# DTUWindEnergy/WindGym

Hardware: AMD Instinct MI355X
Metric: env-steps/sec (whole node), 16-turbine farm x 4096 envs (higher is better)
Workload: dtype f32

## Files before the change

### windgym_amd/csrc/wg_env.hip

```cpp
#include <hip/hip_runtime.h>

#ifndef WG_ENV_ABLATE
#define WG_ENV_ABLATE 0
#endif
#include "wg_env_common.h"
#include "wg_internal.h"

struct __attribute__((aligned(16))) EnvSlotLds {
    int dev_rem, fill_rem, sub, budget;
    double s_new;
    int n_emit, n_valid, new_valid;
    unsigned n_emitted;
    float s_off_f, near_f, move_max, ti_pow;
    double s_off, ws;
    float ws_f, ti_f, wd_env, base_acc;
    int n_pushed, pend_farm_n, pend_base_n, n_flow;
    double c_time;
    int c_head;
    unsigned c_part, c_flow, c_istep, c_tag, n_emitted0;
    float out_pw;
    unsigned c_add;
    int bg_init;
    int pad_[3];
};
static_assert(sizeof(EnvSlotLds) == WG_ENV_SLOT_LDS_BYTES, "keep WG_ENV_SLOT_LDS_BYTES in sync (wg_flow.h)");
#define WG_ENV_OFF_SRC4 0
#define WG_ENV_OFF_REC4 1024
#define WG_ENV_OFF_RING 2048
#define WG_ENV_OFF_XR 3072
#define WG_ENV_OFF_SRC2 3584
#define WG_ENV_OFF_SL 4096
#define WG_ENV_OFF_HDR (WG_ENV_OFF_SL + 4 * WG_ENV_SLOT_LDS_BYTES)
#define WG_ENV_OFF_STAGE (WG_ENV_OFF_HDR + 128)
static_assert(WG_ENV_OFF_STAGE == WG_ENV_FIXED_LDS_BYTES, "keep WG_ENV_FIXED_LDS_BYTES in sync (wg_flow.h)");

__device__ __forceinline__ float env_slot_sums(const float v, const int N, const int NS, const int k, const int tid) {
    if (N == 16) return wg_row_sum(v);
    if (N < 16) {
        const int r = tid >> 4, i = tid & 15;
        const float x = __shfl(v, (r * N + i) & 63, 64);
        const float s = wg_row_sum((i < N && r < NS) ? x : 0.f);
        return __shfl(s, k << 4, 64);
    }
    const int h = tid >> 5, i = tid & 31;
    const float x = __shfl(v, (h * N + i) & 63, 64);
    float s = (i < N && h < NS) ? x : 0.f;
    WG_ROW_REDUCE(s, wg_addf)
    s += __shfl_xor(s, 16, 64);
    return __shfl(s, k << 5, 64);
}

static __device__ __forceinline__ void env_clone_dev(char* const smem, const int kd, const int N, const int P, const double dt_d,
                                                               float* const py_env, unsigned* const ra_env, const unsigned src,
                                                               const unsigned dst, const int lane) {
    float4* const Lsrc4 = reinterpret_cast<float4*>(smem + WG_ENV_OFF_SRC4);
    int4* const Lring = reinterpret_cast<int4*>(smem + WG_ENV_OFF_RING);
    float2* const Lsrc2 = reinterpret_cast<float2*>(smem + WG_ENV_OFF_SRC2);
    EnvSlotLds* const SL = reinterpret_cast<EnvSlotLds*>(smem + WG_ENV_OFF_SL);
    const int ga = (kd - 1) * N, gb = kd * N;
    const int4 last = Lring[ga + N - 1];
    const int nq = (last.x + last.y) >> 2;
    {
        const float4* const ps = reinterpret_cast<const float4*>(py_env + src);
        float4* const pd = reinterpret_cast<float4*>(py_env + dst);
        const uint4* const rs = reinterpret_cast<const uint4*>(ra_env + 2 * (size_t)src);
        uint4* const rd = reinterpret_cast<uint4*>(ra_env + 2 * (size_t)dst);
#pragma unroll 2
        for (int q = lane; q < nq; q += 64) {
            const float4 y = ps[q];
            const uint4 r0 = rs[q], r1 = rs[q + nq];
            pd[q] = y; rd[q] = r0; rd[q + nq] = r1;
        }
    }
    if (lane < N) {
        Lsrc4[gb + lane] = Lsrc4[ga + lane];
        Lsrc2[gb + lane] = Lsrc2[ga + lane];
        Lring[gb + lane].z = Lring[ga + lane].z;
    }
    if (lane == 0) {
        const EnvSlotLds& a = SL[kd - 1];
        EnvSlotLds& b = SL[kd];
        b.n_valid = a.n_valid; b.n_emitted = a.n_emitted; b.s_off = a.s_off;
        b.dev_rem = 0; b.sub = 0;
        b.budget = a.budget;
        double tm = a.c_time;
        for (int i = 0; i < a.n_flow; ++i) tm += dt_d;
        b.c_time = tm;
        int hd = a.c_head + (int)((a.n_emitted - a.n_emitted0) % (unsigned)P); if (hd >= P) hd -= P;
        b.c_head = hd; b.n_emitted0 = a.n_emitted;
        b.c_istep = a.c_istep + (unsigned)a.n_flow;
    }
}

template <bool NOISE, int WPE, int GLUE, int SPLIT>
__device__ __forceinline__ void env_flow(char* const smem, char* const smem_pass, float* const zone, const int wv, const int role, const int mode,
                                         const float* __restrict__ actions, const uint8_t* __restrict__ mask, const int chunk, EnvFlowOut& out) {
    const int tid = threadIdx.x & 63, e = blockIdx.x;
    int N, F, NS, NL;
    float inv_N;
    {
        const KArgsPtr ka = wg_cold_args();
        N = ka->p.N; F = ka->p.F; inv_N = ka->p.inv_N;
        NS = WPE == 2 ? F : 2 * F; NL = NS * N;
    }
    const int kbase = WPE == 2 ? wv * F : 0;
    const bool valid = tid < NL;
    const int g = valid ? tid : 0;
    const int k = (int)(((float)g + 0.5f) * inv_N);
    const int t = g - k * N;
    const int c = WPE == 2 ? wv : (F == 2 ? (k >> 1) : k), farm = F == 2 ? (k & 1) : 0;

    float4* const Lsrc4 = reinterpret_cast<float4*>(smem + WG_ENV_OFF_SRC4);
    uint4* const Lrec4 = reinterpret_cast<uint4*>(smem + WG_ENV_OFF_REC4);
    int4* const Lring = reinterpret_cast<int4*>(smem + WG_ENV_OFF_RING);
    double* const Lxr = reinterpret_cast<double*>(smem + WG_ENV_OFF_XR);
    float2* const Lsrc2 = reinterpret_cast<float2*>(smem + WG_ENV_OFF_SRC2);
    EnvSlotLds* const SL = reinterpret_cast<EnvSlotLds*>(smem + WG_ENV_OFF_SL);
    float* const def = reinterpret_cast<float*>(smem + WG_ENV_OFF_STAGE);
    float* const tiav = def + WG_ENV_CAP;
    unsigned short* const cl = reinterpret_cast<unsigned short*>(tiav + WG_ENV_CAP);
    unsigned short* const ql = reinterpret_cast<unsigned short*>(smem + WG_ENV_OFF_STAGE);
    EnvSlotLds& my = SL[k];

    WG_STAMP(0);
    typedef const __attribute__((address_space(4))) WgEnv* CEnvPtr;
    int env_live;
    bool role_live = false, role_dev = false, defer_init = false, split_on = false;
    bool parked = false;
    float yaw, tu, tti, oyaw;
    {
        const KArgsPtr k0 = wg_cold_args();
        static_assert(sizeof(WgEnv) == 128, "the env header is loaded as 32 words");
        const int hw = reinterpret_cast<const int*>(k0->d.env + e)[tid & 31];
        if (GLUE != 0 && tid < 32) reinterpret_cast<int*>(smem + WG_ENV_OFF_HDR)[tid] = hw;
        out.bg_init_pending = 0; out.rounds = 0; out.first_obs = 0;
        const bool use_mask = mode == WG_MODE_RESET && mask != nullptr;
        const uint8_t mask_byte = *(use_mask ? mask + e : reinterpret_cast<const uint8_t*>(k0->d.env + e));
        const bool masked_out = use_mask && mask_byte == 0;
        const unsigned ctx_id = (unsigned)(e * 2 + c), slot_id = (unsigned)(e * 2 * F + kbase + k);
        const unsigned tb = (unsigned)((e * 2 * F + kbase) * N + g);
        const unsigned tcx = ctx_id * (unsigned)N + (unsigned)t;

        int dev_rem, fill_rem, n_pushed, pend_farm_n, pend_base_n, init_pending, time_max_c, n_valid, c_head;
        unsigned n_emitted, c_part, c_flow, c_istep, c_tag, c_add;
        double s_off, ws, l_xr, l_yr, c_time;
        float ti_f, wd_env, l_yaw, l_u, l_ti, l_act;
        float4 l_bnd;
        int l_roff, l_rnext;
        auto load_state = [&]() __attribute__((always_inline)) {
            const KArgsPtr kl = wg_cold_args();
            const WgSlot& slot = kl->d.slot[slot_id];
            const WgCtx& cx = kl->d.ctx[ctx_id];
            dev_rem = slot.dev_remaining; fill_rem = slot.fill_remaining;
            s_off = slot.s_off; c_time = slot.time; c_head = slot.head; n_valid = slot.n_valid; c_istep = slot.istep;
            n_emitted = slot.n_emitted; c_part = slot.part_count; c_flow = slot.flow_count; c_add = slot.add_count;
            ws = cx.ws; ti_f = (float)cx.ti; wd_env = (float)cx.wd;
            n_pushed = cx.n_pushed; pend_farm_n = cx.pend_farm_n; pend_base_n = cx.pend_base_n;
            c_tag = (unsigned)cx.episode_tag; init_pending = cx.init_pending; time_max_c = cx.time_max;
            const int* ro = kl->d.roff + ctx_id * (unsigned)(N + 1);
            l_roff = ro[(unsigned)t]; l_rnext = ro[(unsigned)t + 1u];
            l_xr = kl->d.xr[tcx]; l_yr = kl->d.yr[tcx];
            l_yaw = kl->d.yaw[tb]; l_u = kl->d.u[tb]; l_ti = kl->d.ti_loc[tb];
            l_bnd = reinterpret_cast<const float4*>(kl->d.bnd)[tb];
        };
        load_state();
        const int n_tab = k0->p.n_tab, S = k0->p.S;
        const unsigned i_tab = (unsigned)min(tid, n_tab - 1), i_s = (unsigned)min(tid, S - 1);
        const float pf_tp = k0->d.tab_power[i_tab], pf_tc = k0->d.tab_ct[i_tab];
        const float pf_dy = k0->d.rotor_dy[i_s], pf_dz = k0->d.rotor_dz[i_s];
        {
            const bool has_act = mode == WG_MODE_STEP && farm == 0;
            const float a = *(has_act ? actions + (unsigned)(e * N + t) : k0->d.tab_ct);
            l_act = has_act ? a : 0.f;
        }

#define WG_HDR_I(f) __builtin_amdgcn_readlane(hw, (int)(offsetof(WgEnv, f) / 4))
        env_live = WG_HDR_I(live);
        int env_done = WG_HDR_I(done), env_shadow_iters = WG_HDR_I(shadow_iters), env_steps_done = WG_HDR_I(steps_done);
        int env_timestep = WG_HDR_I(timestep), env_time_max_live = WG_HDR_I(time_max_live);
#undef WG_HDR_I
        if (SPLIT && role == 1) {
            if (tid == 0) { *reinterpret_cast<int*>(smem + WG_ENV_OFF_HDR) = 0; if (GLUE != 0 && (SPLIT == 1 || wv == 0)) reinterpret_cast<int*>(zone)[LEAN_PRE_FLAG] = 0; }
            asm volatile("s_waitcnt vmcnt(0) lgkmcnt(0)" ::: "memory");
        }
        if (WPE == 2) {
            asm volatile("" : "+s"(env_live), "+s"(env_done), "+s"(env_shadow_iters), "+s"(env_steps_done), "+s"(env_timestep), "+s"(env_time_max_live) : : "memory");
            asm volatile("s_barrier" ::: "memory");
        }
        if (SPLIT && role == 1 && GLUE != 0 && c == env_live) {
            const EnvKArgsPtr kz = (EnvKArgsPtr)wg_cold_args();
            const LeanEarly zr = lean_early_load(*(const WgParams*)&kz->gp, *(const WgPtrs*)&kz->gd, e, N, F, tid, hw);
            double* const zs = reinterpret_cast<double*>(zone);
#pragma unroll
            for (int sI = 0; sI < WG_N_CH; ++sI) { zs[LEAN_PRE_S(sI, tid)] = zr.S[sI]; zone[LEAN_PRE_LV(sI, tid)] = zr.lv[sI]; }
            zone[LEAN_PRE_MET(tid)] = zr.met;
            if (tid == 0) { zone[LEAN_PRE_FOLD] = zr.f_old; zone[LEAN_PRE_BOLD] = zr.b_old; }
            asm volatile("s_waitcnt lgkmcnt(0)" ::: "memory");
            if (tid == 0) env_flag_set(reinterpret_cast<int*>(zone) + LEAN_PRE_FLAG);
        }
        out.env_live = env_live;
        out.truncates = env_timestep >= env_time_max_live;
        out.steps_done = env_steps_done; out.time_max_live = env_time_max_live;

        const bool is_live_c = (c == env_live);
        const int autoreset = k0->p.autoreset;
        int budget = 0;
        long plan_left = 0;
        if (mode == WG_MODE_STEP) {
            role_live = is_live_c && !env_done;
            role_dev = !is_live_c && autoreset != 0;
            const int bg_pending = WPE == 2 ? (is_live_c ? 0 : __shfl(init_pending, 0, 64)) : __shfl(init_pending, (env_live ^ 1) * F * N, 64);
            out.bg_init_pending = autoreset && bg_pending;
            if (SPLIT == 2 && role == 1 && out.bg_init_pending) return;
            if (autoreset && bg_pending && WPE == 1 && !out.truncates) {
                defer_init = true;
                budget = 0;
            } else if (autoreset && bg_pending) {
                const KArgsPtr ki = wg_cold_args();
                const WgParams& gp = *ki->d.gp;
                env_init_episode<GLUE != 0>(e, env_live ^ 1, tid);
                full_barrier<64>();
                load_state();
                const int fill_max = F == 2 ? max(gp.fill_a, gp.fill_b) : gp.fill_a;
                const int tm = WPE == 2 ? ki->d.ctx[e * 2 + env_live].time_max : __shfl(time_max_c, env_live * F * N, 64);
                const long total = wg_rule_episode_steps(tm, gp.extra_inc);
                const int dev0 = __shfl(dev_rem, WPE == 2 ? 0 : (env_live ^ 1) * F * N, 64);
                budget = wg_shadow_share(dev0 + gp.K * fill_max, total - env_steps_done, env_steps_done, e);
                budget = wg_shadow_share(dev_rem + gp.K * fill_rem, total - env_steps_done, env_steps_done, e, farm ? 0x80000000u : 0u);
                plan_left = total - env_steps_done;
            } else {
                const long total = wg_rule_episode_steps_inc(env_time_max_live, k0->p.env_inc);
                budget = role_dev ? wg_shadow_share(dev_rem + k0->p.K * fill_rem, total - env_steps_done, env_steps_done, e, farm ? 0x80000000u : 0u) : 0;
                plan_left = total - env_steps_done;
            }
        } else {
            role_dev = is_live_c && !masked_out;
            budget = chunk;
        }
        bool clone_here = false;
        if (k0->p.env_share) {
            const int dev_a = __shfl(dev_rem, (tid - N) & 63, 64);
            parked = valid && role_dev && farm == 1 && dev_rem > 0 && c_istep == 0u && dev_a > 0;
            const int twin_fill = __shfl(parked ? fill_rem + 1 : 0, (tid + N) & 63, 64);
            const bool lead = valid && role_dev && farm == 0 && twin_fill > 0;
            if (lead && mode == WG_MODE_STEP && !defer_init)
                budget = wg_shadow_share(dev_rem + k0->p.K * max(fill_rem, twin_fill - 1), plan_left, env_steps_done, e);
            if (parked) budget = 0;
            clone_here = lead && budget >= dev_rem;
        }
        if (SPLIT) {
            const bool two = valid && role_dev && budget >= 2;
            split_on = mode == WG_MODE_STEP && k0->p.K == 1 && (is_live_c || (SPLIT == 2 && !out.bg_init_pending)) && !defer_init && !__ballot(two) &&
                       !__ballot(clone_here);
            if (role == 1 && !split_on) return;
        }
        if (WPE == 2 && valid && t == 0) {
            my.dev_rem = dev_rem; my.fill_rem = fill_rem; my.bg_init = out.bg_init_pending; my.n_flow = 0; my.out_pw = 0.f;
        }
        {
            const bool any_work = valid && (role_live || (role_dev && budget > 0 && (dev_rem > 0 || fill_rem > 0)));
            if (!__ballot(any_work)) {
                if (WPE == 2 && mode == WG_MODE_STEP && !is_live_c && autoreset && role == 0) {
                    const int d0 = __shfl(dev_rem, 0, 64), f0 = __shfl(fill_rem, 0, 64), np0 = __shfl(n_pushed, 0, 64);
                    const KArgsPtr kf = wg_cold_args();
                    if (d0 == 0 && f0 == 0 && kf->d.gd->next_obs_ok != nullptr && kf->d.gd->next_obs_ok[ctx_id] == 0) {
                        out.first_obs = 1;
                        env_first_obs<GLUE != 0>((int)ctx_id, np0, tid);
                    }
                }
                return;
            }
        }

        const KArgsPtr k1 = wg_cold_args();
        const int rlen = l_rnext - l_roff;
        const int head = n_emitted == 0u ? rlen - 1 : fast_mod((int)(n_emitted - 1u), rlen, __builtin_amdgcn_rcpf((float)rlen));
        const float ws_f = (float)ws;
        if (valid) {
            Lxr[g] = l_xr;
            Lsrc4[g] = make_float4((float)l_xr, (float)l_yr, l_bnd.y, l_bnd.z);
            Lsrc2[g] = make_float2(l_bnd.x, l_bnd.w);
            Lring[g] = make_int4(l_roff, rlen, head, k);
            Lrec4[g] = make_uint4(0u, 0u, 0u, __float_as_uint(1.f));
            if (t == 0) {
                my.dev_rem = dev_rem; my.fill_rem = fill_rem; my.sub = 0; my.budget = budget;
                my.n_valid = n_valid; my.n_emitted = n_emitted; my.n_emitted0 = n_emitted;
                my.move_max = fabsf(k1->p.hill) * ws_f * k1->p.dt; my.ti_pow = fast_pow(ti_f, k1->p.tic);
                my.s_off = s_off; my.ws = ws; my.ws_f = ws_f; my.ti_f = ti_f; my.wd_env = wd_env; my.base_acc = 0.f;
                my.n_pushed = n_pushed; my.pend_farm_n = pend_farm_n; my.pend_base_n = pend_base_n; my.n_flow = 0;
                my.bg_init = out.bg_init_pending;
                my.c_time = c_time; my.c_head = c_head; my.c_part = c_part; my.c_flow = c_flow; my.c_istep = c_istep; my.c_tag = c_tag; my.c_add = c_add;
            }
        }
        float* const tabp = reinterpret_cast<float*>(smem + k1->p.env_off_tab);
        float* const tabct = tabp + n_tab;
        float2* const rpt = reinterpret_cast<float2*>(tabct + n_tab);
        const float hub = k1->p.hub;
        auto rp = [&](const float dy_, const float dz_) __attribute__((always_inline)) {
            const float dz = hub + dz_ - hub;
            return make_float2(dy_, dz * dz);
        };
        if (tid < n_tab) { tabp[tid] = pf_tp; tabct[tid] = pf_tc; }
        if (tid < S) rpt[tid] = rp(pf_dy, pf_dz);
        for (int i = tid + 64; i < n_tab; i += 64) { tabp[i] = k1->d.tab_power[i]; tabct[i] = k1->d.tab_ct[i]; }
        for (int i = tid + 64; i < S; i += 64) rpt[i] = rp(k1->d.rotor_dy[i], k1->d.rotor_dz[i]);

        yaw = l_yaw; tu = l_u; tti = l_ti; oyaw = l_yaw;
        if (role_live && farm == 0 && valid) {
            yaw = wg_rule_adjust_yaw(k1->p.action_method, yaw, l_act, k1->p.yaw_min, k1->p.yaw_max, k1->p.yaw_step);
        }
    }
    float tpow = 0.f, tct = 0.f, cg = 1.f;
    float sws = 0.f, swd = 0.f, syaw = 0.f, sp_ = 0.f;
    int part_acc = 0, stream_acc = 0;
    bool stepped = false;
    lds_barrier<64>();
    WG_STAMP(1);

    auto glue_early = [&]() __attribute__((always_inline)) {
        if (GLUE != 0 && SPLIT == 0) {
            if (WPE == 2 && wv != env_live) {
                out.g_early = LeanEarly{};
            } else {
                const EnvKArgsPtr kz = (EnvKArgsPtr)wg_cold_args();
                const int hwl = reinterpret_cast<const int*>(smem + WG_ENV_OFF_HDR)[tid & 31];
                out.g_early = lean_early_load(*(const WgParams*)&kz->gp, *(const WgPtrs*)&kz->gd, e, N, F, tid, hwl);
            }
        }
    };
    for (int round = 0;; ++round) {
        bool stepping, is_dev;
        int sub, K;
        if (__ballot(parked)) {
            bool due = parked && SL[k - 1].dev_rem == 0;
            unsigned long long due_m = __ballot(due);
            if (due_m) {
                full_barrier<64>();
                const KArgsPtr kc = wg_cold_args();
                const unsigned pstride = (unsigned)kc->p.pstride;
                const size_t pb_env = (size_t)(e * 2 * F + kbase) * pstride;
                const int src_lane = (tid - N) & 63;
                const float c_tu = __shfl(tu, src_lane, 64), c_tti = __shfl(tti, src_lane, 64), c_pw = __shfl(tpow, src_lane, 64);
                const float c_ct = __shfl(tct, src_lane, 64), c_cg = __shfl(cg, src_lane, 64);
                if (due) { tu = c_tu; tti = c_tti; tpow = c_pw; tct = c_ct; cg = c_cg; stepped = true; parked = false; }
                while (due_m) {
                    const int kd = __builtin_amdgcn_readlane(k, __builtin_ctzll(due_m));
                    env_clone_dev(smem, kd, N, kc->p.P, kc->p.dt_d, kc->d.py + pb_env, kc->d.rec_a + 2 * pb_env, (unsigned)(kd - 1) * pstride,
                                  (unsigned)kd * pstride, tid);
                    due_m &= ~(((1ull << N) - 1ull) << (kd * N));
                }
                lds_barrier<64>();
                glue_early();
            }
        }
        {
            const KArgsPtr kr = wg_cold_args();
            K = kr->p.K;
            const int4 sch = *reinterpret_cast<const int4*>(&my.dev_rem);
            const bool active = sch.x > 0 || sch.y > 0;
            stepping = valid && (role_live ? (round < K) : (role_dev && active && (sch.w > 0 || sch.z != 0)));
            is_dev = !role_live && sch.x > 0;
            sub = sch.z;
            if (!__ballot(stepping)) break;
        out.rounds = round + 1;
            if (round > 0) full_barrier<64>();

            if (role_live && farm == 1 && stepping) {
                const float ystep = kr->p.yaw_step;
                if (kr->p.base_controller == WG_CTRL_LOCAL) {
                    yaw = wg_rule_ctrl_local(yaw, 0.f, ystep);
                } else {
                    yaw = wg_rule_ctrl_global(yaw, ystep);
                }
            }

            if (stepping && t == 0) {
                const double dpart = kr->p.dpart;
                const int P = kr->p.P;
                const double s_off = my.s_off, adv = my.ws * kr->p.dt_d;
                double s_new = s_off + adv;
                int n_emit = 0;
                while (s_new >= dpart) { s_new -= dpart; ++n_emit; }
                if (n_emit > P) n_emit = P;
                int new_valid = my.n_valid + n_emit; if (new_valid > P) new_valid = P;
                my.s_new = s_new; my.n_emit = n_emit; my.new_valid = new_valid;
                my.s_off_f = (float)s_off;
                my.near_f = (float)(s_off + adv + dpart) + 0.01f;
            }
        }
        lds_barrier<64>();
        WG_STAMP(4);

        unsigned cmask = 0u;
        {
            const KArgsPtr kp = wg_cold_args();
            const float D = kp->p.D, inv_D = kp->p.inv_D, eps_max = kp->p.env_eps_max;
            const int gs0 = k * N;
            const float lim0 = kp->p.R_rot + 1.0e-3f * D;
            const float near_f = my.near_f, move_max = my.move_max;
            const float xt_f = Lsrc4[g].x, yt_f = Lsrc4[g].y;
#pragma unroll 4
            for (int s2 = 0; s2 < N; ++s2) {
                const float4 a = Lsrc4[gs0 + s2];
                const float2 b = Lsrc2[gs0 + s2];
                const float dxf = xt_f - a.x;
                const bool nearp = dxf < near_f;
                const float kb_ = nearp ? fmaxf(WG_K_MAX, a.z) : a.z, eb_ = nearp ? fmaxf(eps_max, a.w) : a.w;
                const float sig_max = (kb_ * (dxf * inv_D) + eb_) * D;
                const float bdv = b.x + (((__float_as_uint(b.y) != 0u) | nearp) ? move_max : 0.f);
                const float gap = fabsf(yt_f - a.y) - (5.0f * sig_max + bdv);
                const bool cd = (s2 != t) & (dxf >= 0.f) & (gap <= lim0);
                cmask |= cd ? (1u << s2) : 0u;
            }
            if (!stepping || (SPLIT && role == 1)) cmask = 0u;
        }
        int cbeg, nc;
        {
            const int cnt = __popc(cmask);
            const int inc = wg_wave_scan_i(cnt);
            cbeg = inc - cnt;
            nc = __builtin_amdgcn_readlane(inc, 63);
            unsigned m = cmask;
            int o = cbeg;
            while (m) { cl[o++] = (unsigned short)((g << 5) | __builtin_ctz(m)); m &= m - 1u; }
        }
        lds_barrier<64>();
        WG_STAMP(5);

        struct Cand { uint2 q0, q1; float y0, y1, xd, wgt; int en, jp0; bool ok, rest; };
        float dsum = 0.f, tia_max = 0.f;
        {
            const KArgsPtr kp = wg_cold_args();
            const unsigned pstride = (unsigned)kp->p.pstride;
            const size_t pb_env = (size_t)(e * 2 * F + kbase) * pstride;
            const uint2* const rc_env = reinterpret_cast<const uint2*>(kp->d.rec_a + 2 * pb_env);
            const float* const py_env = kp->d.py + pb_env;
            const double inv_dpart = kp->p.inv_dpart;
            const float inv_D = kp->p.inv_D;
            auto issue = [&](Cand& cd, const int cidx, const int c0, const int c1) __attribute__((always_inline)) {
                cd.ok = false; cd.rest = false;
                if (cidx >= c1) return;
                def[cidx - c0] = 0.f; tiav[cidx - c0] = 0.f;
                const unsigned en = cl[cidx];
                cd.en = (int)en;
                const int gt = (int)(en >> 5);
                const int4 rt = Lring[gt];
                const int gs = rt.w * N + (int)(en & 31u);
                const EnvSlotLds& q = SL[rt.w];
                const double dx = Lxr[gt] - Lxr[gs];
                if (!(dx > 0.0)) return;
                cd.xd = (float)dx * inv_D;
                const double xi = (dx - q.s_new) * inv_dpart;
                const double jf = floor(xi);
                cd.wgt = (float)(xi - jf);
                int j = (int)jf;
                if (j < 0) { j = 0; cd.wgt = 0.f; }
                if (j + 1 > q.new_valid - 1) return;
                const int4 rg = Lring[gs];
                const int Rs = rg.y, hd = rg.z;
                const unsigned mv = __float_as_uint(Lsrc2[gs].y);
                cd.rest = !(mv != 0u && (int)(q.n_emitted - mv) < Rs);
                cd.jp0 = j - q.n_emit;
                int r0 = hd - cd.jp0; if (r0 < 0) r0 += Rs;
                int r1 = hd - cd.jp0 - 1; if (r1 < 0) r1 += Rs;
                if (cd.jp0 < 0) r0 = 0;
                if (cd.jp0 + 1 < 0) r1 = 0;
                const unsigned sb = (unsigned)rg.w * pstride + (unsigned)rg.x;
                cd.q0 = rc_env[sb + (unsigned)r0]; cd.q1 = rc_env[sb + (unsigned)r1];
                cd.y0 = 0.f; cd.y1 = 0.f;
                if (!cd.rest) { cd.y0 = py_env[sb + (unsigned)r0]; cd.y1 = py_env[sb + (unsigned)r1]; }
#if WG_ENV_ABLATE & 1
                cd.q0 = make_uint2(Lrec4[gs].x, Lrec4[gs].y); cd.q1 = cd.q0; cd.y0 = cd.y1 = Lsrc4[gs].y;
#endif
                cd.ok = true;
            };
            Cand ca, cb_;
            issue(ca, tid, 0, min(nc, WG_ENV_CAP));
            WG_STAMP(11);

            if (stepping) {
                const KArgsPtr kq = wg_cold_args();
                const int n_tab = kq->p.n_tab;
                const float* const tabct = reinterpret_cast<const float*>(smem + kq->p.env_off_tab) + n_tab;
                const float gy = yaw * WG_DEG2RAD_F;
                const float sg = __sinf(gy);
                cg = __cosf(gy);
                const float wsn = fmaxf(tu * cg, 0.0f);
                const float ctx = fminf(fmaxf(env_tab(tabct, kq->p.tab_x0, kq->p.tab_inv_dx, n_tab, wsn) * cg * cg, 0.0f), 0.96f);
                const float rq = __builtin_amdgcn_sqrtf(1.0f - ctx);
                const float beta = 0.5f * (1.0f + rq) * __builtin_amdgcn_rcpf(rq);
                const float rk = kq->p.ka * tti + kq->p.kb;
                const float reps = kq->p.eps0 * __builtin_amdgcn_sqrtf(beta);
                const float rhv = -kq->p.hill * sg * tu;
                if (rk > WG_K_MAX || fabsf(rhv) > WG_HV_MAX) atomicOr(kq->d.status, WG_STATUS_BIT_RANGE);
                const unsigned na_ = pack_a(ctx, rk), nb_ = pack_b(tu * __builtin_amdgcn_rcpf(kq->p.ue_scale * my.ws_f), rhv);
                float4 s4 = Lsrc4[g];
                s4.z = fmaxf(s4.z, rk + WG_K_MAX / 65535.0f);
                s4.w = fmaxf(s4.w, reps + 1.0f / 65535.0f);
                Lsrc4[g] = s4;
                const int n_emit = my.n_emit;
                if (n_emit > 0 && rec_moves(nb_)) Lsrc2[g].y = __uint_as_float(my.n_emitted + (unsigned)n_emit);
                Lrec4[g] = make_uint4(na_, nb_, __float_as_uint(tu), __float_as_uint(cg));
            }
            lds_barrier<64>();
            WG_STAMP(2);

            const KArgsPtr ke2 = wg_cold_args();
            const float dpart_f = ke2->p.dpart_f, D = ke2->p.D, dt = ke2->p.dt, R_rot = ke2->p.R_rot, eps0 = ke2->p.eps0, ue_scale = ke2->p.ue_scale;
            const float tia = ke2->p.no_ti_fold ? 0.f : ke2->p.tia, tib = ke2->p.tib, tid_ = ke2->p.tid, inv_S = ke2->p.inv_S;
            const int S = ke2->p.S;
            const float2* const rpt = reinterpret_cast<const float2*>(smem + ke2->p.env_off_tab + 8 * ke2->p.n_tab);
            auto eval_cand = [&](const Cand& cd, const int pos) __attribute__((always_inline)) {
                    if (!cd.ok) return;
#ifdef WG_TIMELINE
                    atomicAdd(&wg_counts[1], 1);
#endif
                    const int gt = cd.en >> 5;
                    const int kt = Lring[gt].w;
                    const int gs = kt * N + (cd.en & 31);
                    const float4 st = Lsrc4[gt];
                    const float ysrc = Lsrc4[gs].y;
                    const EnvSlotLds& q = SL[kt];
                    const int jp0 = cd.jp0, jp1 = jp0 + 1;
                    float py0 = cd.rest ? ysrc : cd.y0, py1 = cd.rest ? ysrc : cd.y1;
                    unsigned a0 = cd.q0.x, b0_ = cd.q0.y, a1 = cd.q1.x, b1_ = cd.q1.y;
                    if (jp0 < 0) {
                        const uint4 rn = Lrec4[gs];
                        py0 = ysrc; a0 = rn.x; b0_ = rn.y;
                        if (jp1 < 0) { py1 = ysrc; a1 = rn.x; b1_ = rn.y; }
                    }
                    const float ue_max = ue_scale * q.ws_f;
                    const float u0 = rec_uf(b0_) * ue_max, u1 = rec_uf(b1_) * ue_max;
                    {
                        const int nv = q.n_valid;
                        const float sof = q.s_off_f;
                        if (!cd.rest && jp0 >= 0 && jp0 < nv) py0 = m0_advect(py0, a0, b0_, jp0, sof, dpart_f, inv_D, dt, eps0);
                        if (!cd.rest && jp1 >= 0 && jp1 < nv) py1 = m0_advect(py1, a1, b1_, jp1, sof, dpart_f, inv_D, dt, eps0);
                    }
                    const float wgt = cd.wgt;
                    const float w0 = 1.0f - wgt, w1 = wgt;
                    const float yc = w0 * py0 + w1 * py1;
                    const float kv = w0 * rec_k(a0) + w1 * rec_k(a1);
                    const float epv = w0 * rec_eps(a0, eps0) + w1 * rec_eps(a1, eps0);
                    const float xd = cd.xd;
                    const float sp = kv * xd + epv;
                    const float sig = sp * D;
                    const float yt = st.y;
                    const float rc2 = (yt - yc) * (yt - yc);
                    const float rcut = R_rot + 5.0f * sig;
                    if (rc2 > rcut * rcut) return;
#ifdef WG_TIMELINE
                    atomicAdd(&wg_counts[2], 1);
                    if (rc2 <= (R_rot + 3.0f * sig) * (R_rot + 3.0f * sig)) atomicAdd(&wg_counts[3], 1);
#endif
                    const float ctv = w0 * rec_ct(a0) + w1 * rec_ct(a1);
                    const float uev = w0 * u0 + w1 * u1;
                    const float inv2s2 = __builtin_amdgcn_rcpf(2.0f * sig * sig);
                    const float cf = m0_cfrac(ctv, sp);
                    const float ind = 0.5f * (1.0f - __builtin_amdgcn_sqrtf(1.0f - ctv));
                    tiav[pos] = tia * fast_pow(ind, tib) * q.ti_pow * fast_pow(fmaxf(xd, 1.0f), tid_) * __expf(-rc2 * inv2s2);
                    const float cgt = __uint_as_float(Lrec4[gt].w), amp = uev * cf;
                    const float ninv = -inv2s2;
                    float acc = 0.f;
#pragma unroll 4
                    for (int sI = 0; sI < ((WG_ENV_ABLATE & 8) ? 1 : S); ++sI) {
                        const float2 rp = rpt[sI];
                        const float dy = yt + rp.x * cgt - yc;
                        acc += amp * __expf((dy * dy + rp.y) * ninv);
                    }
                    def[pos] = acc * inv_S;
            };
#ifdef WG_TIMELINE
            if (tid == 0) atomicAdd(&wg_counts[0], nc);
#endif
            for (int c0 = 0; c0 < nc; c0 += WG_ENV_CAP) {
                const int c1 = min(nc, c0 + WG_ENV_CAP);
                if (c0 > 0) { lds_barrier<64>(); issue(ca, c0 + tid, c0, c1); }
                for (int cb = c0; cb < c1; cb += 64) {
                    cb_ = ca;
                    issue(ca, cb + 64 + tid, c0, c1);
                    eval_cand(cb_, cb - c0 + tid);
                }
                lds_barrier<64>();
                if (stepping) {
                    const int b0 = max(cbeg, c0), b1 = min(cbeg + __popc(cmask), c1);
                    for (int cc = b0; cc < b1; ++cc) {
                        dsum += def[cc - c0];
                        tia_max = fmaxf(tia_max, tiav[cc - c0]);
                    }
                }
            }
        }
        if (SPLIT && split_on && role == 0) {
            __builtin_amdgcn_s_waitcnt(0x0070);
            if (tid == 0) env_flag_set(reinterpret_cast<int*>(smem_pass + WG_ENV_OFF_HDR));
            if (stepping) {
                const int4 rg = Lring[g];
                const unsigned mvl = __float_as_uint(Lsrc2[g].y);
                const int n_emit = my.n_emit;
                const bool full = (mvl != 0u && (int)(my.n_emitted - mvl) < rg.y) || n_emit >= 4 || n_emit >= rg.y;
                stream_acc += full ? rg.y : n_emit;
            }
        }
        if (stepping) {
            const float ti_f = my.ti_f;
            tu = my.ws_f;
            tu -= dsum;
            tti = __builtin_amdgcn_sqrtf(ti_f * ti_f + tia_max * tia_max);
        }
        lds_barrier<64>();
        WG_STAMP(9);

        if (!(SPLIT && split_on && role == 0)) {
            const KArgsPtr kp = wg_cold_args();
            const unsigned pstride = (unsigned)kp->p.pstride;
            const size_t pb_env = (size_t)(e * 2 * F + kbase) * pstride;
            float* const py_env = kp->d.py + pb_env;
            unsigned* const ra_env = kp->d.rec_a + 2 * pb_env;
            int nlist;
            {
                int cnt = 0, nqd = 0;
                bool full = false;
                if (stepping) {
                    const int4 rg = Lring[g];
                    const int rlen = rg.y, n_emit = my.n_emit;
                    const unsigned mvl = __float_as_uint(Lsrc2[g].y);
                    nqd = rlen >> 2;
                    const bool moving = mvl != 0u && (int)(my.n_emitted - mvl) < rlen;
                    full = moving || n_emit >= 4 || n_emit >= rlen;
                    stream_acc += full ? rlen : n_emit;
                    if (full) cnt = nqd;
                    else if (n_emit > 0) {
                        const unsigned sb = (unsigned)k * pstride + (unsigned)rg.x;
                        const uint4 rn = Lrec4[g];
                        const float y0 = Lsrc4[g].y;
#pragma unroll
                        for (int em = 0; em < 3; ++em) {
                            if (em < n_emit) {
                                int r = rg.z + 1 + em; if (r >= rlen) r -= rlen;
                                const unsigned ix = sb + (unsigned)r;
                                py_env[ix] = y0;
                                reinterpret_cast<uint2*>(ra_env)[ix] = make_uint2(rn.x, rn.y);
                            }
                        }
                    }
                }
                const int inc = wg_wave_scan_i(cnt);
                nlist = (WG_ENV_ABLATE & 2) ? 0 : __builtin_amdgcn_readlane(inc, 63);
                if (full) {
                    const int base = inc - cnt;
                    const unsigned tag = (unsigned)g << 10;
                    for (int i = 0; i < nqd; ++i) ql[base + i] = (unsigned short)(tag | (unsigned)i);
                }
            }
            lds_barrier<64>();
            WG_STAMP(10);
#ifdef WG_TIMELINE
            if (tid == 0) atomicAdd(&wg_counts[4], nlist);
#endif

            const float dpart_f = kp->p.dpart_f, inv_D = kp->p.inv_D, dt = kp->p.dt, eps0 = kp->p.eps0;
            struct QuadReq { float4 py; uint4 ra, rb; int g, kq; unsigned q; };
            auto request = [&](QuadReq& r, const int cidx) __attribute__((always_inline)) {
                const bool v = cidx < nlist;
                const unsigned en = v ? ql[cidx] : 0u;
                r.g = (int)(en >> 10); r.kq = (int)(en & 1023u);
                const int4 rg = Lring[r.g];
                r.q = (((unsigned)rg.w * pstride + (unsigned)rg.x) >> 2) + (unsigned)r.kq;
                if (v) {
                    r.py = reinterpret_cast<const float4*>(py_env)[r.q];
                    r.ra = reinterpret_cast<const uint4*>(ra_env)[2u * r.q];
                    r.rb = reinterpret_cast<const uint4*>(ra_env)[2u * r.q + 1u];
                }
            };
            auto advect_quad = [&](const QuadReq& cur, const int cidx) __attribute__((always_inline)) {
                if (cidx >= nlist) return;
                const int gq = cur.g, kq = cur.kq;
                const unsigned q = cur.q;
                const int4 rg = Lring[gq];
                const EnvSlotLds& sl = SL[rg.w];
                const int n_emit_q = sl.n_emit, n_valid_q = sl.n_valid;
                const float sof = sl.s_off_f;
                const int R = rg.y, hd = rg.z;
                const int r0 = 4 * kq;
                int j0 = hd - r0; if (j0 < 0) j0 += R;
                int e0 = r0 - hd - 1; if (e0 < 0) e0 += R;
                const bool emits = (e0 < n_emit_q) || (n_emit_q > 0 && e0 + 3 >= R);
                float pyv[4] = {cur.py.x, cur.py.y, cur.py.z, cur.py.w};
                unsigned rav[4] = {cur.ra.x, cur.ra.z, cur.rb.x, cur.rb.z};
                unsigned rbv[4] = {cur.ra.y, cur.ra.w, cur.rb.y, cur.rb.w};
#pragma unroll
                for (int i = 0; i < 4; ++i) {
                    int j = j0 - i; if (j < 0) j += R;
                    const float adv = m0_advect(pyv[i], rav[i], rbv[i], j, sof, dpart_f, inv_D, dt, eps0);
                    pyv[i] = j < n_valid_q ? adv : pyv[i];
                }
                const float y0 = Lsrc4[gq].y;
                if (emits) {
                    const uint4 rn = Lrec4[gq];
#pragma unroll
                    for (int i = 0; i < 4; ++i) {
                        int ei = e0 + i; if (ei >= R) ei -= R;
                        if (ei < n_emit_q) {
                            pyv[i] = y0; rav[i] = rn.x; rbv[i] = rn.y;
                        }
                    }
                    reinterpret_cast<uint4*>(ra_env)[2u * q] = make_uint4(rav[0], rbv[0], rav[1], rbv[1]);
                    reinterpret_cast<uint4*>(ra_env)[2u * q + 1u] = make_uint4(rav[2], rbv[2], rav[3], rbv[3]);
                }
                reinterpret_cast<float4*>(py_env)[q] = make_float4(pyv[0], pyv[1], pyv[2], pyv[3]);
                float ex = 0.f;
#pragma unroll
                for (int i = 0; i < 4; ++i) {
                    int j = j0 - i; if (j < 0) j += R;
                    if (j < n_valid_q) ex = fmaxf(ex, fabsf(pyv[i] - y0));
                }
                if (ex > Lsrc2[gq].x) atomicMax(reinterpret_cast<int*>(&Lsrc2[gq].x), __float_as_int(ex));
            };
            QuadReq qa, qb;
            qa.py = qb.py = make_float4(0.f, 0.f, 0.f, 0.f); qa.ra = qa.rb = qb.ra = qb.rb = make_uint4(0u, 0u, 0u, 0u);
            request(qa, tid);
            if (SPLIT && role == 1) {
                if (!env_flag_wait(reinterpret_cast<int*>(smem + WG_ENV_OFF_HDR))) atomicOr(kp->d.status, WG_STATUS_BIT_STATE);
            }
            for (int base = 0; base < nlist; base += 64) {
                qb = qa;
                request(qa, base + 64 + tid);
                advect_quad(qb, base + tid);
            }
        }
        lds_barrier<64>();
        WG_STAMP(3);
        if (SPLIT && role == 1) {
            if (stepping) reinterpret_cast<float4*>(wg_cold_args()->d.bnd)[(unsigned)((e * 2 * F + kbase) * N + g)].x = Lsrc2[g].x;
            return;
        }
        glue_early();

        const bool measuring = stepping && !is_dev;
        const bool unit_end = measuring && (sub + 1 == K);
        const KArgsPtr kc = wg_cold_args();
        const float inv_k = 1.0f / (float)K;
        const unsigned ctx_id = (unsigned)(e * 2 + c);
        if (stepping) {
            {
                int4 rg = Lring[g];
                const int n_emit = my.n_emit;
                rg.z += n_emit;
                if (n_emit >= rg.y) rg.z %= rg.y; else if (rg.z >= rg.y) rg.z -= rg.y;
                Lring[g].z = rg.z;
                part_acc += min(my.new_valid, rg.y);
            }
            stepped = true;
            const int n_tab = kc->p.n_tab;
            const float tab_x0 = kc->p.tab_x0, tab_inv_dx = kc->p.tab_inv_dx;
            const float* const tabp = reinterpret_cast<const float*>(smem + kc->p.env_off_tab);
            const float wsn = fmaxf(tu * cg, 0.0f);
            tpow = env_tab(tabp, tab_x0, tab_inv_dx, n_tab, wsn);
            tct = env_tab(tabp + n_tab, tab_x0, tab_inv_dx, n_tab, wsn) * cg * cg;
            if (measuring && farm == 0) {
                const float wsm = __builtin_amdgcn_sqrtf(tu * tu);
                const float wdm = 0.f + my.wd_env;
                float val[WG_N_CH] = {sws + wsm, swd + wdm, syaw + yaw, sp_ + tpow};
                if (unit_end) {
                    const int n_pushed = my.n_pushed;
                    const unsigned tcx = ctx_id * (unsigned)N + (unsigned)t;
                    kc->d.cur_ws[tcx] = wsm;
                    kc->d.cur_wd[tcx] = wdm;
                    if (K != 1) {
#pragma unroll
                        for (int ch = 0; ch < WG_N_CH; ++ch) val[ch] *= inv_k;
                    }
                    if (NOISE) {
                        const uint64_t noise_key = ((CEnvPtr)(kc->d.env + e))->noise_key;
                        const uint32_t episode_tag = my.c_tag;
#pragma unroll
                        for (int ch = 0; ch < WG_N_CH; ++ch)
                            if (kc->p.noise_sigma[ch] != 0.f)
                                val[ch] += kc->p.noise_sigma[ch] * wg_noise_normal(noise_key, (uint32_t)n_pushed, (uint32_t)t,
                                                                                   (uint32_t)ch, episode_tag);
                    }
                    float* __restrict__ rbase = kc->d.ring + (size_t)ctx_id * kc->p.ring_stride;
#pragma unroll
                    for (int ch = 0; ch < WG_N_CH; ++ch) {
                        const int H = kc->p.hlen[ch];
                        rbase[(unsigned)(kc->p.ring_off[ch] + fast_mod(n_pushed, H, kc->p.inv_hlen[ch]) * N + t)] = val[ch];
                    }
                    if (GLUE != 0) {
#pragma unroll
                        for (int ch = 0; ch < WG_N_CH; ++ch) out.g_nw[ch] = val[ch];
                    }
                    sws = val[0]; swd = val[1]; sp_ = val[3];
                } else {
                    sws = val[0]; swd = val[1]; syaw = val[2]; sp_ = val[3];
                }
            }
        }
        float a_ws = 0.f, a_wd = 0.f, a_pw = 0.f;
        if (__ballot(measuring)) {
            a_ws = env_slot_sums((measuring && farm == 0) ? sws : 0.f, N, NS, k, tid);
            a_wd = env_slot_sums((measuring && farm == 0) ? swd : 0.f, N, NS, k, tid);
            a_pw = env_slot_sums(measuring ? (farm == 0 ? sp_ : tpow) : 0.f, N, NS, k, tid);
        }
        if (stepping && t == 0) {
            const int n_emit = my.n_emit;
            my.n_valid = my.new_valid; my.s_off = my.s_new; my.n_emitted += (unsigned)n_emit;
            my.n_flow += 1; my.budget -= 1;
            float base_acc = my.base_acc;
            if (measuring && farm == 1) base_acc += a_pw;
            if (unit_end) {
                const FlowP __attribute__((address_space(4)))& pc = kc->p;
                if (farm == 0) {
                    const int n_pushed = my.n_pushed, pend_farm_n = my.pend_farm_n;
                    float* fbase = kc->d.fring + (size_t)ctx_id * pc.fring_stride;
                    fbase[pc.fring_off[WG_CH_WS] + umod_small(n_pushed, pc.hlen[WG_CH_WS], pc.hmagic[WG_CH_WS])] = a_ws * pc.inv_N;
                    fbase[pc.fring_off[WG_CH_WD] + umod_small(n_pushed, pc.hlen[WG_CH_WD], pc.hmagic[WG_CH_WD])] = a_wd * pc.inv_N;
                    fbase[pc.fring_off[WG_CH_POWER] + umod_small(n_pushed, pc.hlen[WG_CH_POWER], pc.hmagic[WG_CH_POWER])] = a_pw;
                    my.out_pw = a_pw;
                    if (role_live) kc->d.step_farm_pow[e] = a_pw;
                    else {
                        kc->d.pend_farm[(size_t)ctx_id * pc.power_avg + umod_small(pend_farm_n, pc.power_avg, pc.pavg_magic)] = a_pw;
                        my.pend_farm_n = pend_farm_n + 1;
                    }
                    my.n_pushed = n_pushed + 1;
                } else {
                    const float bp = K == 1 ? base_acc : base_acc * inv_k;
                    my.out_pw = bp;
                    if (role_live) kc->d.step_base_pow[e] = bp;
                    else {
                        const int pend_base_n = my.pend_base_n;
                        kc->d.pend_base[(size_t)ctx_id * pc.power_avg + umod_small(pend_base_n, pc.power_avg, pc.pavg_magic)] = bp;
                        my.pend_base_n = pend_base_n + 1;
                    }
                    base_acc = 0.f;
                }
            }
            my.base_acc = base_acc;
            if (is_dev) my.dev_rem -= 1;
            else if (sub + 1 >= K) { my.sub = 0; if (!role_live) my.fill_rem -= 1; }
            else my.sub = sub + 1;
        }
        if (unit_end && farm == 0) { sws = 0.f; swd = 0.f; syaw = 0.f; sp_ = 0.f; }
        lds_barrier<64>();
        WG_STAMP(6);
    }

    WG_STAMP(7);
    const KArgsPtr ke = wg_cold_args();
    const float part_slot = env_slot_sums((float)part_acc, N, NS, k, tid);
    const float stream_slot = env_slot_sums((float)stream_acc, N, NS, k, tid);
    if (valid && stepped) {
        const unsigned tb = (unsigned)((e * 2 * F + kbase) * N + g);
        const float4 s4 = Lsrc4[g];
        const float2 s2 = Lsrc2[g];
        ke->d.yaw[tb] = yaw; ke->d.u[tb] = tu; ke->d.v[tb] = 0.f; ke->d.w[tb] = 0.f;
        ke->d.ti_loc[tb] = tti; ke->d.power[tb] = tpow; ke->d.ct[tb] = tct;
        if (SPLIT && split_on) {
            float4* const bp = reinterpret_cast<float4*>(ke->d.bnd) + tb;
            bp->y = s4.z; bp->z = s4.w; bp->w = s2.y;
        } else reinterpret_cast<float4*>(ke->d.bnd)[tb] = make_float4(s2.x, s4.z, s4.w, s2.y);
        if (role_live && farm == 0) ke->d.old_yaw[(unsigned)(e * N + t)] = oyaw;
        if (t == 0) {
            const int n_flow = my.n_flow, P = ke->p.P;
            const double dt_d = ke->p.dt_d;
            double tm = my.c_time;
            for (int i = 0; i < n_flow; ++i) tm += dt_d;
            const unsigned n_emitted = my.n_emitted;
            int hd = my.c_head + (int)((n_emitted - my.n_emitted0) % (unsigned)P); if (hd >= P) hd -= P;
            WgSlot& slot = ke->d.slot[(unsigned)(e * 2 * F + kbase + k)];
            slot.part_count = my.c_part + (unsigned)part_slot;
            slot.add_count = my.c_add + (unsigned)stream_slot;
            slot.head = hd; slot.n_valid = my.n_valid; slot.s_off = my.s_off; slot.time = tm;
            slot.istep = my.c_istep + (unsigned)n_flow; slot.n_emitted = n_emitted;
            slot.dev_remaining = my.dev_rem; slot.fill_remaining = my.fill_rem;
            slot.flow_count = my.c_flow + (unsigned)n_flow;
            WgCtx& cx = ke->d.ctx[(unsigned)(e * 2 + c)];
            if (farm == 0) { cx.n_pushed = my.n_pushed; cx.pend_farm_n = my.pend_farm_n; }
            if (farm == F - 1) cx.pend_base_n = my.pend_base_n;
        }
    }
    if (GLUE != 0) {
        out.g_yaw = yaw; out.g_old = oyaw; out.g_pw = tpow;
        out.g_pwb = F == 2 ? __shfl(tpow, min(tid + N, 63), 64) : 0.f;
    }
    WG_STAMP(8);
    if (mode == WG_MODE_STEP && (WPE == 1 || c != env_live) && !defer_init) {
        const EnvSlotLds& bs = SL[WPE == 2 ? 0 : (env_live ^ 1) * F];
        const int bctx = e * 2 + (env_live ^ 1);
        bool build = false;
        if (ke->p.autoreset && bs.dev_rem == 0 && bs.fill_rem == 0)
            build = bs.n_flow == 0 ? (ke->d.gd->next_obs_ok != nullptr && ke->d.gd->next_obs_ok[bctx] == 0) : out.truncates != 0;
        if (build) {
            const int np = bs.n_pushed;
            out.first_obs = 1;
            full_barrier<64>();
            env_first_obs<GLUE != 0>(bctx, np, tid);
            glue_early();
        }
    }
    if (defer_init) {
        env_init_episode<GLUE != 0>(e, env_live ^ 1, tid);
        full_barrier<64>();
        if (valid && t == 0 && c != env_live) {
            const WgSlot& slot = ke->d.slot[(unsigned)(e * 2 * F + kbase + k)];
            my.dev_rem = slot.dev_remaining; my.fill_rem = slot.fill_remaining;
        }
        lds_barrier<64>();
        glue_early();
    }
}


template <bool NOISE, int GLUE, int WPE, int SPLIT = 0>
__global__ void __launch_bounds__(64 * (WPE + SPLIT), WG_ENV_WAVES)
k_flow_env(const FlowP p_, const FlowPtrs d_, const int mode, const float* __restrict__ actions,
           const uint8_t* __restrict__ mask, const int chunk, const WgParams gp_, const WgPtrs gd_,
           float* __restrict__ obs_out, float* __restrict__ reward_out, uint8_t* __restrict__ trunc_out,
           float* __restrict__ final_obs_out) {
    extern __shared__ __attribute__((aligned(16))) char smem[];
#ifdef WG_TIMELINE
    if (threadIdx.x == 0) { for (int i = 0; i < 20; ++i) wg_stamps[i] = 0; wg_stamps[14] = wall_clock64(); for (int i = 0; i < 8; ++i) wg_counts[i] = 0; }
    __syncthreads();
#endif
    const int wv4 = WPE == 2 ? __builtin_amdgcn_readfirstlane((int)(threadIdx.x >> 6)) : 0;
    int wv = wv4, role = 0;
    if (SPLIT == 1 && wv4 == 2) {
        role = 1;
        wv = __builtin_amdgcn_readfirstlane(reinterpret_cast<const int*>(wg_cold_args()->d.env + blockIdx.x)[offsetof(WgEnv, live) / 4]) & 1;
    }
    if (SPLIT == 2) { wv = wv4 & 1; role = wv4 >> 1; }
    const int lds_wave = WPE == 2 ? wg_cold_args()->p.env_lds : 0;
    char* const sm = smem + wv4 * lds_wave;
    char* const sm_pass = smem + (SPLIT == 2 ? 2 + wv : 2) * lds_wave;
    float* const zone = SPLIT ? reinterpret_cast<float*>(smem + (2 + SPLIT) * lds_wave) : nullptr;
    EnvFlowOut fo;
    env_flow<NOISE, WPE, GLUE, SPLIT>(sm, sm_pass, zone, wv, role, mode, actions, mask, chunk, fo);
    if (SPLIT && role == 1) {
        if (GLUE != 0 && fo.truncates) { __builtin_amdgcn_s_waitcnt(0x0070); __syncthreads(); }
        return;
    }
    if (GLUE != 0) {
        if (SPLIT != 0 || fo.truncates) full_barrier<64>();
        if (WPE == 2) {
            if (wv != fo.env_live) {
                const EnvKArgsPtr kb = (EnvKArgsPtr)wg_cold_args();
                const int e = (int)blockIdx.x;
                if (kb->p.autoreset && !fo.truncates && (threadIdx.x & 63) == 0) {
                    const int F = kb->p.F, K = kb->p.K;
                    const EnvSlotLds* const SLb = reinterpret_cast<const EnvSlotLds*>(sm + WG_ENV_OFF_SL);
                    int work = 0;
                    for (int f = 0; f < F; ++f) work = max(work, SLb[f].dev_rem + K * SLb[f].fill_rem);
                    env_bg_plan(kb, work, fo, e);
                }
                if (fo.bg_init_pending && (threadIdx.x & 63) == 0) kb->d.ctx[e * 2 + wv].init_pending = 0;
                if (fo.truncates) __builtin_amdgcn_s_waitcnt(0x0070);
            }
            if (fo.truncates) __syncthreads();
        }
        if (WPE == 1 || wv == fo.env_live) {
            const EnvKArgsPtr kg = (EnvKArgsPtr)wg_cold_args();
            const int F = kg->p.F, K = kg->p.K;
            const EnvSlotLds* const SLa = reinterpret_cast<const EnvSlotLds*>(sm + WG_ENV_OFF_SL);
            const int la = WPE == 2 ? 0 : fo.env_live * F, lb = (fo.env_live ^ 1) * F;
            const float fp = SLa[la].out_pw, bp = F == 2 ? SLa[la + 1].out_pw : 0.f;
            int work = 0;
            if (WPE == 1) for (int f = 0; f < F; ++f) work = max(work, SLa[lb + f].dev_rem + K * SLa[lb + f].fill_rem);
            const int hw = reinterpret_cast<const int*>(sm + WG_ENV_OFF_HDR)[threadIdx.x & 31];
            LeanFused fz;
            fz.pre = nullptr; fz.regs = SPLIT == 0; fz.early = SPLIT == 0;
            if (SPLIT == 0) fz.ev = fo.g_early;
            if (SPLIT) {
                if (!env_flag_wait(reinterpret_cast<int*>(zone) + LEAN_PRE_FLAG)) atomicOr(kg->d.status, WG_STATUS_BIT_STATE);
                fz.pre = zone;
            }
            int gl = (int)(threadIdx.x & 63);
            asm volatile("" : "+v"(gl));
            const int own = gl < kg->p.N ? gl : 0;
            if (WPE == 2) {
#pragma unroll
                for (int ch = 0; ch < WG_N_CH; ++ch) fz.nw[ch] = __shfl(fo.g_nw[ch], own, 64);
                fz.yaw = fo.g_yaw; fz.old_yaw = fo.g_old; fz.pw = fo.g_pw; fz.pwb = fo.g_pwb;
            } else {
                const int src = fo.env_live * F * kg->p.N + own;
#pragma unroll
                for (int ch = 0; ch < WG_N_CH; ++ch) fz.nw[ch] = __shfl(fo.g_nw[ch], src, 64);
                fz.yaw = __shfl(fo.g_yaw, src, 64); fz.old_yaw = __shfl(fo.g_old, src, 64);
                fz.pw = __shfl(fo.g_pw, src, 64); fz.pwb = __shfl(fo.g_pwb, src, 64);
            }
            WG_STAMP(12);
            env_glue<GLUE, WPE>(kg, fz, fp, bp, work, fo, hw, gl);
            WG_STAMP(13);
        }
    }
#ifdef WG_TIMELINE
    {
        const KArgsPtr kt = wg_cold_args();
        if (threadIdx.x == 0 && kt->d.dbg) {
            wg_stamps[15] = wall_clock64();
            long long* row = kt->d.dbg + (size_t)blockIdx.x * 32;
            for (int kq = 0; kq < 16; ++kq) row[kq] = wg_stamps[kq];
            row[16] = fo.bg_init_pending; row[17] = fo.rounds; row[18] = fo.first_obs;
            row[19] = GLUE != 0 ? (long long)kt->d.env[blockIdx.x].timestep : 0;
            for (int kq = 0; kq < 8; ++kq) row[20 + kq] = wg_counts[kq];
            for (int kq = 0; kq < 4; ++kq) row[28 + kq] = wg_stamps[16 + kq];
        }
    }
#endif
}

template <bool NZ, int G>
static EnvKernel env_kernel(const int wpe, const int split) {
    if constexpr (G != 0) {
        if (split == 2) return k_flow_env<NZ, G, 2, 2>;
        if (split == 1) return k_flow_env<NZ, G, 2, 1>;
    }
    return wpe == 2 ? k_flow_env<NZ, G, 2> : k_flow_env<NZ, G, 1>;
}
static void env_launch(const FlowP* p, const FlowPtrs* d, const int glue, const int mode, const float* actions, const uint8_t* mask,
                       const int chunk, const WgParams* gp, const WgPtrs* gd, float* obs, float* reward, uint8_t* trunc,
                       float* final_obs, hipStream_t st) {
    const int wpe = p->env_wpe == 2 ? 2 : 1;
    const int split = glue != 0 && wpe == 2 && (p->env_split == 1 || p->env_split == 2) ? p->env_split : 0;
    const size_t lds = (size_t)p->env_lds * (wpe + split) + (split ? LEAN_PRE_BYTES : 0);
    const EnvKernel k = glue == 2 ? (p->noise ? env_kernel<true, 2>(wpe, split) : env_kernel<false, 2>(wpe, split))
                      : glue == 1 ? (p->noise ? env_kernel<true, 1>(wpe, split) : env_kernel<false, 1>(wpe, split))
                                  : (p->noise ? env_kernel<true, 0>(wpe, split) : env_kernel<false, 0>(wpe, split));
    hipLaunchKernelGGL(k, dim3(p->B), dim3(64 * (wpe + split)), lds, st, *p, *d, mode, actions, mask, chunk, *gp, *gd, obs, reward, trunc, final_obs);
}

extern "C" void wg_launch_flow_env(const FlowP* p, const FlowPtrs* d, int mode, const float* actions, const uint8_t* mask,
                                   int chunk, hipStream_t st) {
    static const WgParams gp0{};
    static const WgPtrs gd0{};
    env_launch(p, d, 0, mode, actions, mask, chunk, &gp0, &gd0, nullptr, nullptr, nullptr, nullptr, st);
}

extern "C" void wg_launch_step_env(const FlowP* p, const FlowPtrs* d, const WgParams* gp, const WgPtrs* gd, const float* actions,
                                   float* obs, float* reward, uint8_t* trunc, float* final_obs, hipStream_t st) {
    env_launch(p, d, gd->multi_out ? 2 : 1, WG_MODE_STEP, actions, nullptr, 0, gp, gd, obs, reward, trunc, final_obs, st);
}
```

### windgym_amd/csrc/wg_flow.h

```cpp
#pragma once
#include "wg_state.h"

#ifndef WG_BOX_WAVES
#define WG_BOX_WAVES 2
#endif
#ifndef WG_FLOW_WAVES_GL
#define WG_FLOW_WAVES_GL 4
#endif
#ifndef WG_FLOW_WAVES
#define WG_FLOW_WAVES 5
#endif
#ifndef WG_FLOW_WAVES_LF
#define WG_FLOW_WAVES_LF 3
#endif
#define WG_LF_OFF_TM(n) (16 * (size_t)(n))
#define WG_LF_OFF_BASE(n) (32 * (size_t)(n))
#define WG_LF_OFF_CL(n) ((36 * (size_t)(n) + 4 * 8 + 15) & ~(size_t)15)
#define WG_LF_OFF_DEF(n) ((WG_LF_OFF_CL(n) + (size_t)(n) * ((n) - 1) + 15) & ~(size_t)15)

struct FlowP {
    int B, N, F, K, P, S, S_pad, S_shift, NP, n_tab;
    int autoreset, action_method, base_controller, power_avg, script_rows, noise;
    int block;
    int res;
    int pstride;
    int target_chunk;
    int lf_cap;
    int lds_off_turb, lds_off_tab, lds_bytes;
    int rec_il;
    int gl;
    int lds_off_ql, lds_off_gat;
    int ql_shift;
    int ql_lpt_shift;
    int envw, env_lds, env_off_tab;
    int env_cap, envb_off_cl;
    int env_wpe;
    int env_split;
    int env_fused;
    int env_inc;
    float env_eps_max;
    float dt, D, inv_D, hub, dpart_f, R_rot, inv_N, inv_S, inv_P;
    int env_share;
    double dt_d, dpart, inv_dpart;
    float yaw_min, yaw_max, yaw_step;
    float ka, kb, eps0, hill, tia, tib, tic, tid;
    float ue_scale;
    float tab_x0, tab_inv_dx;
    int hlen[WG_N_CH], ring_off[WG_N_CH], fring_off[WG_N_CH];
    float inv_hlen[WG_N_CH], inv_power_avg;
    unsigned hmagic[WG_N_CH], pavg_magic;
    int ring_stride, fring_stride;
    float noise_sigma[WG_N_CH];
    int turb_mode, bnx, bny, bnz, box_pow2;
    int coarse, cnx, cny, cnz, cbox_pow2;
    long long box_cells, cbox_cells;
    double inv_bdx, inv_bdy, inv_bdz, fc_scale, D_d, hub_d;
    float inv_sqrt_S;
    int added, anx, any, anz, abox_pow2;
    int no_ti_fold, deficit_model;
    float km1, km2r;
    float sg_af, sg_bf, sg_cf;
    double inv_adx, inv_ady, inv_adz;
    double inv_bn[3], inv_an[3];
    int an_ct, an_ti, an_x, an_r;
    float an_ct0, an_inv_dct, an_lti0, an_inv_dlti, an_inv_dx, an_inv_dr, an_inv_ka;
};

struct FlowPtrs {
    float *py, *pz, *vlp, *wlp;
    unsigned *rec_a, *rec_b;
    const float4* box4;
    const float4* box4c;
    const float4* abox4;
    const float4* box8;
    const float4* abox8;
    const float* dtab;
    float *yaw, *u, *v, *w, *ti_loc, *power, *ct;
    float* bnd;
    WgSlot* slot;
    WgCtx* ctx;
    const WgEnv* env;
    const double *xr, *yr;
    const int* jneed;
    const int* roff;
    const uint8_t* qown;
    int* status;
    float *ring, *fring, *cur_ws, *cur_wd, *pend_farm, *pend_base, *old_yaw, *step_farm_pow, *step_base_pow;
    const float *rotor_dy, *rotor_dz, *tab_power, *tab_ct;
    const float *script_uvw, *script_power;
    long long* dbg;
    const WgParams* gp;
    const WgPtrs* gd;
    WgEnv* env_rw;
};

#define WG_ENV_SLOT_LDS_BYTES 160
#define WG_ENV_FIXED_LDS_BYTES (3 * 64 * 16 + 2 * 64 * 8 + 4 * WG_ENV_SLOT_LDS_BYTES + 128)
#define WG_ENV_CAP 256
#define LEAN_PRE_BYTES 3584
#define WG_ENVB_FIXED_LDS_BYTES(nlp) ((93 + 48) * (nlp) + 4 * 208 + 128)
#define WG_TURB_LDS_BYTES 120
#define WG_GAT_BYTES (2 * 64 * 16 + 2 * 64 * 4)
#define WG_MASK_WORDS 4
```

### windgym_amd/csrc/wg_glue_lean.h

```cpp
#pragma once
#include <hip/hip_runtime.h>

#include "wg_device.h"
#include "wg_obs.h"

__device__ inline float deque_at(const float* dq, int n_total, int maxlen, int q) {
    const int n = n_total < maxlen ? n_total : maxlen;
    return dq[(n_total - n + q) % maxlen];
}

struct EnvHot {
    int live, timestep, episode, done, shadow_iters, farm_pow_n, base_pow_n, steps_done;
    float ep_return, ep_power_sum;
    int ep_len;
};
__device__ inline EnvHot env_load(const WgEnv& env) {
    EnvHot h;
    h.live = env.live; h.timestep = env.timestep; h.episode = env.episode; h.done = env.done;
    h.shadow_iters = env.shadow_iters; h.farm_pow_n = env.farm_pow_n; h.base_pow_n = env.base_pow_n;
    h.steps_done = env.steps_done; h.ep_return = env.ep_return; h.ep_power_sum = env.ep_power_sum; h.ep_len = env.ep_len;
    return h;
}
__device__ inline void env_writeback(WgEnv& env, const EnvHot& ev, const int lane, const bool skip_shadow = false) {
    if (lane == 0) env.live = ev.live;
    if (lane == 1) env.timestep = ev.timestep;
    if (lane == 2) env.episode = ev.episode;
    if (lane == 3) env.done = ev.done;
    if (lane == 4 && !skip_shadow) env.shadow_iters = ev.shadow_iters;
    if (lane == 5) env.farm_pow_n = ev.farm_pow_n;
    if (lane == 6) env.base_pow_n = ev.base_pow_n;
    if (lane == 7) env.steps_done = ev.steps_done;
    if (lane == 8) env.ep_return = ev.ep_return;
    if (lane == 9) env.ep_power_sum = ev.ep_power_sum;
    if (lane == 10) env.ep_len = ev.ep_len;
}

struct LeanArgs { WgParams p; WgPtrs d; };
typedef const __attribute__((address_space(4))) LeanArgs* LeanArgsPtr;

template <bool MULTI, typename P, typename D>
__device__ __forceinline__ void lean_swap_fast(const P& p, const D& d, const int e, const int live, const int lane, const float fp,
                                       const float bp, const int fslot, const int bslot, const int n1f, const int n1b,
                                       const int episode_next, float* obs, float* om, const int pfn, const int pbn,
                                       const int nnp, const int time_max, const float rated) {
    const int nctx = e * 2 + (live ^ 1);
    const int F = p.F, PA = p.power_avg, obs_dim = p.obs_dim;
    float* fq = d.farm_pow + (size_t)e * PA;
    float* bq = d.base_pow + (size_t)e * PA;
    const float* pf = d.pend_farm + (size_t)nctx * PA;
    const float* pb = d.pend_base + (size_t)nctx * PA;
    const float* no = d.next_obs + (size_t)nctx * obs_dim;
    WgEnv& envw = d.env[e];
    const int mf = pfn < PA ? pfn : PA, mb = pbn < PA ? pbn : PA;
    const int n2f = n1f + mf, n2b = n1b + mb;
    const int i = lane < PA ? lane : 0;
    int qf = (i - n1f) % PA; if (qf < 0) qf += PA;
    int qb = (i - n1b) % PA; if (qb < 0) qb += PA;
    const float f_old = fq[i], f_new = deque_at(pf, pfn > 0 ? pfn : 1, PA, qf < mf ? qf : 0);
    const float b_old = F == 2 ? bq[i] : 0.f, b_new = F == 2 ? deque_at(pb, pbn > 0 ? pbn : 1, PA, qb < mb ? qb : 0) : 0.f;
    float ov[4];
#pragma unroll
    for (int k = 0; k < 4; ++k) ov[k] = lane + 64 * k < obs_dim ? no[lane + 64 * k] : 0.f;
    bool unready = false;
    if (lane < F) { const WgSlot& sl = d.slot[nctx * F + lane]; unready = sl.dev_remaining != 0 || sl.fill_remaining != 0; }
    const wg_u128 r_state = envw.rng_state, r_inc = envw.rng_inc;
    const uint32_t r_has32 = envw.rng_has32, r_u32 = envw.rng_u32;
    const int tobs = p.turb_obs, odm = p.obs_dim_multi;
    auto put = [&](const int k, const float v) {
        obs[k] = v;
        if (MULTI && om) { const int t = k / tobs; om[(size_t)t * odm + (k - t * tobs)] = v; }
    };
#pragma unroll
    for (int k = 0; k < 4; ++k) if (lane + 64 * k < obs_dim) put(lane + 64 * k, ov[k]);
    for (int k = lane + 256; k < obs_dim; k += WG_WAVE) put(k, no[k]);
    double sf = 0.0, sb = 0.0;
    {
        float vf = lane == fslot ? fp : f_old;
        if (lane < PA && qf < mf) { vf = f_new; fq[lane] = vf; }
        if (lane < (n2f < PA ? n2f : PA)) sf = (double)vf;
        if (F == 2) {
            float vb = lane == bslot ? bp : b_old;
            if (lane < PA && qb < mb) { vb = b_new; bq[lane] = vb; }
            if (lane < (n2b < PA ? n2b : PA)) sb = (double)vb;
        }
    }
#pragma unroll
    for (int s2 = 32; s2 > 0; s2 >>= 1) { sf += __shfl_xor(sf, s2, 64); sb += __shfl_xor(sb, s2, 64); }
    if (unready) atomicOr(d.status, WG_STATUS_BIT_STATE);
    if (lane == 0) {
        WgCtx& ncx = d.ctx[nctx];
        WgCtx& rcx = d.ctx[e * 2 + live];
        ncx.pend_farm_n = 0; ncx.pend_base_n = 0;
        d.next_obs_ok[nctx] = 0;
        rcx.init_pending = 1;
        rcx.episode_tag = episode_next;
        rcx.snap_state = r_state; rcx.snap_inc = r_inc;
        rcx.snap_has32 = r_has32; rcx.snap_u32 = r_u32;
    }
    if (lane == 0) envw.live = live ^ 1;
    if (lane == 1) envw.timestep = 0;
    if (lane == 2) envw.steps_done = 0;
    if (lane == 3) envw.farm_pow_n = n2f;
    if (lane == 4) envw.base_pow_n = n2b;
    if (lane == 5) envw.time_max_live = time_max;
    if (lane == 6) envw.rated_live = rated;
    if (lane == 7) envw.fsum_run = sf;
    if (lane == 8) envw.bsum_run = sb;
    if (lane == 9) envw.n_pushed_live = nnp;
    if (lane == 10) envw.shadow_iters = 0;
    return;
}

template <bool MULTI, bool GEN>
__device__ __attribute__((noinline)) void lean_swap(const WgParams* gp, const WgPtrs* gd, const int e, const int live, const int lane,
                                                    const float fp, const float bp, const int fslot, const int bslot,
                                                    const int n1f, const int n1b, const int episode_next, float* obs, float* om,
                                                    float* mscr, const int pfn, const int pbn, const int nnp, const int time_max,
                                                    const float rated, const bool prepared, const LeanArgsPtr ka) {
    const int nctx = e * 2 + (live ^ 1);
    const WgParams& p = *gp;
    const WgPtrs& d = *gd;
    const int N = p.N, F = p.F, PA = p.power_avg, NS = N + 1;
    WgCtx& ncx = d.ctx[nctx];
    if (lane < F) {
        const WgSlot& sl = d.slot[nctx * F + lane];
        if (sl.dev_remaining != 0 || sl.fill_remaining != 0) atomicOr(d.status, WG_STATUS_BIT_STATE);
    }
    const int mf = pfn < PA ? pfn : PA, mb = pbn < PA ? pbn : PA;
    float* fq = d.farm_pow + (size_t)e * PA;
    float* bq = d.base_pow + (size_t)e * PA;
    const float* pf = d.pend_farm + (size_t)nctx * PA;
    const float* pb = d.pend_base + (size_t)nctx * PA;
    const int n2f = n1f + mf, n2b = n1b + mb;
    double sf = 0.0, sb = 0.0;
    for (int i = lane; i < PA; i += WG_WAVE) {
        int qf = (i - n1f) % PA; if (qf < 0) qf += PA;
        float vf = i == fslot ? fp : fq[i];
        if (qf < mf) { vf = deque_at(pf, pfn, PA, qf); fq[i] = vf; }
        if (i < (n2f < PA ? n2f : PA)) sf += (double)vf;
        if (F == 2) {
            int qb = (i - n1b) % PA; if (qb < 0) qb += PA;
            float vb = i == bslot ? bp : bq[i];
            if (qb < mb) { vb = deque_at(pb, pbn, PA, qb); bq[i] = vb; }
            if (i < (n2b < PA ? n2b : PA)) sb += (double)vb;
        }
    }
    bool obs_done = false;
    if (prepared) {
        if (lane == 0) d.next_obs_ok[nctx] = 0;
        if (!MULTI && !GEN && obs) {
            const float* no = d.next_obs + (size_t)nctx * p.obs_dim;
            for (int i = lane; i < p.obs_dim; i += WG_WAVE) obs[i] = no[i];
            obs_done = true;
        }
    } else {
        int Lg = 1;
        while (Lg < 8 && N * (Lg * 2) <= WG_WAVE) Lg *= 2;
        const int sub = lane & (Lg - 1), per_pass = WG_WAVE / Lg;
        const bool farm_ent = GEN && p.sum_mask_f != 0u;
        for (int t0 = 0; t0 < N + (farm_ent ? 1 : 0); t0 += per_pass) {
            const int ent = t0 + lane / Lg;
            const bool have = ent < N || (ent == N && farm_ent);
            const SumsEnt q = wg_sums_ent(p, d, nctx, have ? ent : 0);
            double* ws_ = d.wsum + (size_t)nctx * WG_N_SUMS * NS + (have ? ent : 0);
            float* o = (obs && !GEN && have) ? obs + (size_t)ent * p.turb_obs : nullptr;
            float* o_m = (MULTI && om && !GEN && have) ? om + (size_t)ent * p.obs_dim_multi : nullptr;
            int n = 0;
#pragma nounroll
            for (int sl = 0; sl < (GEN ? WG_N_SUMS : WG_N_CH); ++sl) {
                const bool on = have && ((q.sm >> sl) & 1u);
                const int ch = sl < WG_N_CH ? sl : WG_CH_WS;
                const int off = q.farm ? p.fring_off[ch] : p.ring_off[ch];
                const int cap = p.ring_cap[ch];
                const int cnt = p.sum_w[sl] < nnp ? p.sum_w[sl] : nnp;
                const int r0 = (nnp - cnt) % cap;
                const bool cur_on = o && ((p.oc.cur_mask >> ch) & 1u) && nnp > 0;
                const float cv = cur_on ? q.rb[off + ((nnp - 1) % cap) * q.stride] : 0.f;
                double acc = 0.0;
                if (on) {
#pragma nounroll
                    for (int k = sub; k < cnt; k += 8 * Lg) {
                        float v[8];
#pragma unroll
                        for (int u = 0; u < 8; ++u) {
                            int row = r0 + min(k + u * Lg, cnt - 1); if (row >= cap) row -= cap;
                            v[u] = q.rb[off + row * q.stride];
                        }
#pragma unroll
                        for (int u = 0; u < 8; ++u)
                            if (k + u * Lg < cnt) acc += sl == WG_SUM_TI2 ? (double)v[u] * (double)v[u] : (double)v[u];
                    }
                }
                for (int s2 = 1; s2 < Lg; s2 <<= 1) acc += __shfl_xor(acc, s2, 64);
                if (on && sub == 0) ws_[(size_t)sl * NS] = acc;
                if (o && sub == 0 && nnp > 0) {
                    if (cur_on) { const float v = wg_scale_r(cv, p.oc.mn[ch], p.oc.inv_rng[ch]); o[n] = v; if (o_m) o_m[n] = v; ++n; }
                    if ((p.oc.rol_mask >> ch) & 1u) {
                        const float v = wg_scale_r(wg_sums_mean(p.oc, acc, ch, nnp), p.oc.mn[ch], p.oc.inv_rng[ch]);
                        o[n] = v; if (o_m) o_m[n] = v; ++n;
                    }
                }
            }
        }
        obs_done = !GEN;
    }
#pragma unroll
    for (int s2 = 32; s2 > 0; s2 >>= 1) { sf += __shfl_xor(sf, s2, 64); sb += __shfl_xor(sb, s2, 64); }
    if (lane == 0) {
        ncx.pend_farm_n = 0; ncx.pend_base_n = 0;
        WgCtx& rcx = d.ctx[e * 2 + live];
        const WgEnv& env = d.env[e];
        rcx.init_pending = 1;
        rcx.episode_tag = episode_next;
        rcx.snap_state = env.rng_state; rcx.snap_inc = env.rng_inc;
        rcx.snap_has32 = env.rng_has32; rcx.snap_u32 = env.rng_u32;
    }
    WgEnv& envw = d.env[e];
    if (lane == 0) envw.live = live ^ 1;
    if (lane == 1) envw.timestep = 0;
    if (lane == 2) envw.steps_done = 0;
    if (lane == 3) envw.farm_pow_n = n2f;
    if (lane == 4) envw.base_pow_n = n2b;
    if (lane == 5) envw.time_max_live = time_max;
    if (lane == 6) envw.rated_live = rated;
    if (lane == 7) envw.fsum_run = sf;
    if (lane == 8) envw.bsum_run = sb;
    if (lane == 9) envw.n_pushed_live = nnp;
    if (lane == 10) envw.shadow_iters = 0;
    if (!obs_done && obs) {
        asm volatile("s_waitcnt vmcnt(0)" ::: "memory");
        auto ld = [&](const int ent) {
            ObsIn o;
            const SumsEnt q = wg_sums_ent(p, d, nctx, ent);
            const double* ws_ = d.wsum + (size_t)nctx * WG_N_SUMS * NS + ent;
#pragma unroll
            for (int sl = 0; sl < WG_N_SUMS; ++sl) o.S[sl] = ((q.sm >> sl) & 1u) ? __builtin_nontemporal_load(ws_ + (size_t)sl * NS) : 0.0;
#pragma unroll
            for (int ch = 0; ch < WG_N_CH; ++ch) {
                const int off = q.farm ? p.fring_off[ch] : p.ring_off[ch];
                o.cur[ch] = (nnp > 0 && ((q.cm >> ch) & 1u)) ? q.rb[off + ((nnp - 1) % p.ring_cap[ch]) * q.stride] : 0.f;
            }
            return o;
        };
        build_obs_sums<MULTI, GEN>(p, lane, obs, nullptr, om, nnp, mscr, ld(lane < N ? lane : 0), ld);
    }
}


#ifndef WG_LEAN_ABLATE
#define WG_LEAN_ABLATE 0
#endif
__device__ __forceinline__ int wg_uni(const int v) { return __builtin_amdgcn_readfirstlane(v); }
__device__ __forceinline__ float wg_uni(const float v) { return __int_as_float(__builtin_amdgcn_readfirstlane(__float_as_int(v))); }

struct LeanEarly {
    double S[WG_N_CH];
    float lv[WG_N_CH], f_old, b_old, met;
};
__device__ __forceinline__ LeanEarly lean_early_load(const WgParams& p, const WgPtrs& d, const int e, const int N, const int F,
                                                     const int lane, const int hw) {
#define WG_HDR_Z(f) __builtin_amdgcn_readlane(hw, (int)(offsetof(WgEnv, f) / 4))
    const int z_live = WG_HDR_Z(live), z_np = WG_HDR_Z(n_pushed_live), z_fn = WG_HDR_Z(farm_pow_n), z_bn = WG_HDR_Z(base_pow_n);
#undef WG_HDR_Z
    const int PA = p.power_avg;
    const SumsRaw zr = wg_sums_load<false, false, true>(p, d, e, e * 2 + z_live, lane < N ? lane : 0, z_np);
    LeanEarly q;
#pragma unroll
    for (int s = 0; s < WG_N_CH; ++s) { q.S[s] = zr.S[s]; q.lv[s] = zr.lv[s]; }
    q.f_old = d.farm_pow[(size_t)e * PA + z_fn % PA];
    q.b_old = F == 2 ? d.base_pow[(size_t)e * PA + z_bn % PA] : 0.f;
    q.met = lane < WG_N_METRICS ? d.metrics[(size_t)e * WG_N_METRICS + lane] : 0.f;
    return q;
}

struct LeanFused {
    float fp, bp;
    int work;
    int bg_init_pending;
    int plan_elsewhere;
    int hw;
    const float* pre;
    int regs;
    float nw[WG_N_CH], yaw, old_yaw, pw, pwb;
    int early;
    LeanEarly ev;
};
#define LEAN_PRE_S(s, lane) ((s) * 64 + (lane))
#define LEAN_PRE_LV(s, lane) (512 + (s) * 64 + (lane))
#define LEAN_PRE_MET(lane) (768 + (lane))
#define LEAN_PRE_FOLD 832
#define LEAN_PRE_BOLD 833
#define LEAN_PRE_FLAG 834

template <bool MULTI, bool GEN, bool FUSED>
__device__ __forceinline__ void lean_step(const WgParams& p, const WgPtrs& d, const WgParams* gp, const WgPtrs* gd, const int e,
                                          const int lane, float* __restrict__ obs_out, float* __restrict__ reward_out,
                                          uint8_t* __restrict__ trunc_out, float* __restrict__ final_obs_out, float* const mscr,
                                          const LeanFused& fz) {
    const int N = p.N, F = p.F, PA = p.power_avg;
    WgEnv& env = d.env[e];
    float* obs = obs_out ? obs_out + (size_t)e * p.obs_dim : nullptr;
    float* om = MULTI ? d.multi_out + (size_t)e * N * p.obs_dim_multi : nullptr;
    float* omf = (MULTI && d.multi_fin) ? d.multi_fin + (size_t)e * N * p.obs_dim_multi : nullptr;
    float* fq = d.farm_pow + (size_t)e * PA;
    float* bq = d.base_pow + (size_t)e * PA;
    const int own = lane < N ? lane : 0;

    static_assert(sizeof(WgEnv) == 128, "lean_step loads the env header as 32 words");
    const int hw = FUSED ? fz.hw : reinterpret_cast<const int*>(&env)[lane & 31];
#define WG_HDR_I(f) __builtin_amdgcn_readlane(hw, (int)(offsetof(WgEnv, f) / 4))
#define WG_HDR_F(f) __int_as_float(WG_HDR_I(f))
#define WG_HDR_D(f) __hiloint2double(__builtin_amdgcn_readlane(hw, (int)(offsetof(WgEnv, f) / 4) + 1), WG_HDR_I(f))
    if (WG_HDR_I(done)) {
        if (lane == 0) atomicOr(d.status, WG_STATUS_BIT_STATE);
        return;
    }
    EnvHot ev;
    ev.live = WG_HDR_I(live); ev.timestep = WG_HDR_I(timestep); ev.episode = WG_HDR_I(episode); ev.done = 0; ev.shadow_iters = 0;
    ev.farm_pow_n = WG_HDR_I(farm_pow_n); ev.base_pow_n = WG_HDR_I(base_pow_n); ev.steps_done = WG_HDR_I(steps_done);
    ev.ep_return = WG_HDR_F(ep_return); ev.ep_power_sum = WG_HDR_F(ep_power_sum); ev.ep_len = WG_HDR_I(ep_len);
    int time_max = WG_HDR_I(time_max_live), n_pushed_live = WG_HDR_I(n_pushed_live);
    float rated_power = WG_HDR_F(rated_live);
    double fsum_run = WG_HDR_D(fsum_run), bsum_run = WG_HDR_D(bsum_run);
#undef WG_HDR_D
#undef WG_HDR_F
#undef WG_HDR_I
    const int live = ev.live, nxt = live ^ 1;
#if defined(WG_TIMELINE) && defined(WG_STAMP2)
    if (FUSED) WG_STAMP2(16);
#endif
    const int ctx_id = e * 2 + live;
    if (WG_LEAN_ABLATE == 1) { if (lane == 0 && reward_out) reward_out[e] = (float)(fsum_run + bsum_run) + (float)(ev.timestep + ev.episode + time_max + n_pushed_live); return; }
    int nx_pfn = 0, nx_pbn = 0, nx_np = 0, nx_tmax = 0;
    float nx_rated = 0.f;
    bool nx_prep = false;
    if (ev.timestep >= time_max && p.autoreset) {
        const WgCtx& nc = d.ctx[e * 2 + nxt];
        nx_pfn = wg_uni(nc.pend_farm_n); nx_pbn = wg_uni(nc.pend_base_n); nx_np = wg_uni(nc.n_pushed); nx_tmax = wg_uni(nc.time_max);
        nx_rated = wg_uni(nc.rated_power);
        nx_prep = d.next_obs_ok != nullptr && wg_uni(d.next_obs_ok[e * 2 + nxt]) != 0;
    }
    const bool pre = FUSED && !GEN && fz.pre != nullptr;
    const bool regs = FUSED && !GEN && !pre && fz.regs != 0;
    const bool early = regs && fz.early != 0;
    SumsRaw raw;
    const bool have2 = !FUSED && lane + WG_WAVE < N;
    SumsRaw raw2 = {};
    const size_t tb_a = (size_t)(ctx_id * F) * N;
    float l_yaw = 0.f, l_old = 0.f, l_pow = 0.f, l_powb = 0.f;
    const float fp = FUSED ? fz.fp : wg_uni(d.step_farm_pow[e]);
    const float bp = F == 2 ? (FUSED ? fz.bp : wg_uni(d.step_base_pow[e])) : 0.f;
    const int fslot = ev.farm_pow_n % PA, bslot = ev.base_pow_n % PA;
    float* met = d.metrics + (size_t)e * WG_N_METRICS;
    float f_old, b_old, l_met;
    if (pre) {
        const double* const zs = reinterpret_cast<const double*>(fz.pre);
#pragma unroll
        for (int s = 0; s < WG_N_SUMS; ++s) { raw.S[s] = 0.0; raw.lv[s] = 0.f; }
#pragma unroll
        for (int s = 0; s < WG_N_CH; ++s) {
            if ((p.sum_mask_t >> s) & 1u) { raw.S[s] = zs[LEAN_PRE_S(s, lane)]; raw.lv[s] = fz.pre[LEAN_PRE_LV(s, lane)]; }
        }
        f_old = wg_uni(fz.pre[LEAN_PRE_FOLD]); b_old = F == 2 ? wg_uni(fz.pre[LEAN_PRE_BOLD]) : 0.f;
        l_met = lane < WG_N_METRICS ? fz.pre[LEAN_PRE_MET(lane)] : 0.f;
    } else if (early) {
#pragma unroll
        for (int s = 0; s < WG_N_SUMS; ++s) { raw.S[s] = 0.0; raw.lv[s] = 0.f; }
#pragma unroll
        for (int s = 0; s < WG_N_CH; ++s) { raw.S[s] = fz.ev.S[s]; raw.lv[s] = fz.ev.lv[s]; }
        f_old = wg_uni(fz.ev.f_old); b_old = F == 2 ? wg_uni(fz.ev.b_old) : 0.f;
        l_met = fz.ev.met;
    } else {
        raw = regs ? wg_sums_load<GEN, false>(p, d, e, ctx_id, own, n_pushed_live) : wg_sums_load<GEN>(p, d, e, ctx_id, own, n_pushed_live);
        if (have2) raw2 = wg_sums_load<GEN>(p, d, e, ctx_id, lane + WG_WAVE, n_pushed_live);
        if (!regs && lane < N) {
            l_yaw = d.yaw[tb_a + lane]; l_old = d.old_yaw[(size_t)e * N + lane]; l_pow = d.power[tb_a + lane];
            if (F == 2) l_powb = d.power[tb_a + N + lane];
        }
        f_old = wg_uni(fq[fslot]); b_old = F == 2 ? wg_uni(bq[bslot]) : 0.f;
        l_met = lane < WG_N_METRICS ? met[lane] : 0.f;
    }
    if (pre || regs) {
        const unsigned msk = p.sum_mask_t | p.cur_mask_t;
#pragma unroll
        for (int ch = 0; ch < WG_N_CH; ++ch) raw.nw[ch] = ((msk >> ch) & 1u) ? fz.nw[ch] : 0.f;
        if (lane < N) { l_yaw = fz.yaw; l_old = fz.old_yaw; l_pow = fz.pw; if (F == 2) l_powb = fz.pwb; }
    }
    int work = 0;
    if (p.autoreset) {
        if (FUSED) {
            work = fz.work;
            if (fz.bg_init_pending && lane == 0) d.ctx[e * 2 + nxt].init_pending = 0;
        } else {
            const WgSlot* const bs = d.slot + (size_t)(e * 2 + nxt) * F;
            for (int f = 0; f < F; ++f) work = max(work, wg_uni(bs[f].dev_remaining) + p.K * wg_uni(bs[f].fill_remaining));
            if (wg_uni(d.ctx[e * 2 + nxt].init_pending) && lane == 0) d.ctx[e * 2 + nxt].init_pending = 0;
        }
    }
#if defined(WG_TIMELINE) && defined(WG_STAMP2)
    if (FUSED) { __builtin_amdgcn_s_waitcnt(0); WG_STAMP2(17); }
#endif
    if (WG_LEAN_ABLATE == 2) {
        float acc = raw.nw[0] + raw.nw[2] + raw.lv[0] + raw.lv[2] + (float)raw.S[0] + (float)raw.S[2] + l_yaw + l_old + l_pow + l_powb + fp + bp + f_old + b_old + l_met;
        if (reward_out) reward_out[e] = acc + (float)work;
        return;
    }

    const bool f_full = ev.farm_pow_n >= PA, b_full = ev.base_pow_n >= PA;
    fsum_run += (double)fp - (f_full ? (double)f_old : 0.0);
    if (F == 2) bsum_run += (double)bp - (b_full ? (double)b_old : 0.0);
    ev.farm_pow_n++;
    if (F == 2) ev.base_pow_n++;
    const int nf = ev.farm_pow_n < PA ? ev.farm_pow_n : PA, nb = ev.base_pow_n < PA ? ev.base_pow_n : PA;
    if (lane == 0) {
        fq[fslot] = fp;
        if (F == 2) bq[bslot] = bp;
        if (fp != fp) atomicOr(d.status, WG_STATUS_BIT_NAN_POWER);
    }
    const int truncated = ev.timestep >= time_max;
    const bool swap_obs = truncated && p.autoreset;
    float* fin = final_obs_out ? final_obs_out + (size_t)e * p.obs_dim : nullptr;
    const int np_step = n_pushed_live;
    n_pushed_live += 1;
    if (WG_LEAN_ABLATE == 3) {
        float acc = raw.nw[0] + raw.nw[2] + raw.lv[0] + raw.lv[2] + (float)raw.S[0] + (float)raw.S[2] + l_yaw + l_old + l_pow + l_powb + l_met;
        if (reward_out) reward_out[e] = acc + (float)work + (float)(fsum_run + bsum_run) + (float)(nf + nb);
        return;
    }

    float pen_s = 0.f, pnow = 0.f, pbase = 0.f;
    if (lane < N) {
        pen_s = p.penalty_type == WG_PEN_CHANGE ? wg_rule_penalty_term(WG_PEN_CHANGE, l_old, l_yaw) : wg_rule_penalty_term(WG_PEN_TOTAL, 0.f, l_yaw);
        pnow = l_pow; pbase = l_powb;
    }
    for (int t = lane + WG_WAVE; t < N; t += WG_WAVE) {
        const float y = d.yaw[tb_a + t];
        pen_s += p.penalty_type == WG_PEN_CHANGE ? wg_rule_penalty_term(WG_PEN_CHANGE, d.old_yaw[(size_t)e * N + t], y)
                                                 : wg_rule_penalty_term(WG_PEN_TOTAL, 0.f, y);
        pnow += d.power[tb_a + t];
        if (F == 2) pbase += d.power[tb_a + N + t];
    }
    if (p.action_penalty >= WG_PENALTY_SWITCH) pen_s = N <= 16 ? wg_row_sum(pen_s) : wg_wave_sum(pen_s);
    pnow = N <= 16 ? wg_row_sum(pnow) : wg_wave_sum(pnow);
    if (F == 2) pbase = N <= 16 ? wg_row_sum(pbase) : wg_wave_sum(pbase);
    pen_s = __shfl(pen_s, 0, 64); pnow = __shfl(pnow, 0, 64); pbase = __shfl(pbase, 0, 64);

    double pr = 0.0;
    switch (p.reward_mode) {
    case WG_REW_BASELINE: pr = (fsum_run * (double)nb) / (bsum_run * (double)nf) - 1.0; break;
    case WG_REW_POWER_AVG: pr = fsum_run / ((double)nf * (double)N * (double)rated_power); break;
    case WG_REW_NONE: pr = 0.0; break;
    case WG_REW_POWER_DIFF: {
        const int wsz = PA / 10;
        double fl = 0.0, fo = 0.0;
        int nl = 0, no = 0;
        for (int i = lane; i < PA; i += WG_WAVE) {
            const float fv = i == fslot ? fp : fq[i];
            if (i < nf) {
                int q = i - (ev.farm_pow_n - nf) % PA; if (q < 0) q += PA;
                if (q >= PA - wsz && q < PA) { fl += (double)fv; nl++; }
                if (q < wsz) { fo += (double)fv; no++; }
            }
        }
#pragma unroll
        for (int o = 32; o > 0; o >>= 1) {
            fl += __shfl_xor(fl, o, 64); fo += __shfl_xor(fo, o, 64);
            nl += __shfl_xor(nl, o, 64); no += __shfl_xor(no, o, 64);
        }
        pr = (fl / (double)nl - fo / (double)no) / N;
        break;
    }
    }
    const float reward = wg_rule_reward(pr, p.power_scaling, wg_rule_penalty(p.action_penalty, p.penalty_type, pen_s, N, p.yaw_max_d));
    ev.timestep += 1 + (p.extra_inc ? 1 : 0);
    ev.steps_done += 1;
    ev.ep_return += reward; ev.ep_power_sum += pnow; ev.ep_len += 1;
    if (lane == 0) {
        if (reward_out) reward_out[e] = reward;
        if (trunc_out) trunc_out[e] = (uint8_t)truncated;
        d.last_pow_agent[e] = pnow; d.last_pow_base[e] = pbase;
    }
    if (lane < WG_N_METRICS) {
        met[lane] = l_met + wg_rule_metric_add(lane, reward, pnow, pbase, truncated, ev.ep_return, ev.ep_len, ev.ep_power_sum);
    }
#if defined(WG_TIMELINE) && defined(WG_STAMP2)
    if (FUSED) WG_STAMP2(18);
#endif
    if (WG_LEAN_ABLATE == 4) {
        float acc = raw.nw[0] + raw.nw[2] + raw.lv[0] + raw.lv[2] + (float)raw.S[0] + (float)raw.S[2];
        if (trunc_out && acc == 123.f) trunc_out[e] = 7;
        return;
    }
    if (truncated) {
        ev.ep_return = 0.f; ev.ep_power_sum = 0.f; ev.ep_len = 0;
        ev.episode += 1;
        if (!p.autoreset) {
            ev.done = 1;
        } else {
        }
    }
    {
        float* o1 = swap_obs ? ((MULTI && omf && !fin) ? obs : fin) : obs;
        if (o1) {
            auto get = [&](const int ent) {
                if (have2 && ent == lane + WG_WAVE) return wg_sums_apply<GEN>(p, d, ctx_id, ent, raw2, !swap_obs);
                return wg_sums_apply<GEN>(p, d, ctx_id, ent, wg_sums_load<GEN>(p, d, e, ctx_id, ent, np_step), !swap_obs);
            };
            const ObsIn oi = wg_sums_apply<GEN>(p, d, ctx_id, own, raw, lane < N && !swap_obs);
            build_obs_sums<MULTI, GEN>(p, lane, o1, swap_obs ? nullptr : fin, swap_obs ? omf : om, np_step + 1, mscr, oi, get,
                                       swap_obs ? nullptr : omf);
        }
    }
#if defined(WG_TIMELINE) && defined(WG_STAMP2)
    if (FUSED) WG_STAMP2(19);
#endif
    if (WG_LEAN_ABLATE == 5) return;

    if (!p.autoreset || truncated) ev.shadow_iters = 0;
    else if (work == 0) ev.shadow_iters = 0;
    else {
        const long total = wg_rule_episode_steps(time_max, p.extra_inc);
        ev.shadow_iters = wg_shadow_share(work, total - ev.steps_done, ev.steps_done, e);
    }
    env_writeback(env, ev, lane, FUSED && fz.plan_elsewhere && !truncated);
    if (lane == 11) env.time_max_live = time_max;
    if (lane == 12) env.rated_live = rated_power;
    if (lane == 13) env.fsum_run = fsum_run;
    if (lane == 14) env.bsum_run = bsum_run;
    if (lane == 15) env.n_pushed_live = n_pushed_live;
    if (swap_obs) {
        if (!GEN && nx_prep && obs && PA <= WG_WAVE)
            lean_swap_fast<MULTI>(p, d, e, live, lane, fp, bp, fslot, bslot, ev.farm_pow_n, ev.base_pow_n, ev.episode + 1, obs, om,
                                  nx_pfn, nx_pbn, nx_np, nx_tmax, nx_rated);
        else
            lean_swap<MULTI, GEN>(gp, gd, e, live, lane, fp, bp, fslot, bslot, ev.farm_pow_n, ev.base_pow_n, ev.episode + 1, obs, om, mscr,
                                  nx_pfn, nx_pbn, nx_np, nx_tmax, nx_rated, nx_prep, (LeanArgsPtr)__builtin_amdgcn_kernarg_segment_ptr());
    }
}
```

### windgym_amd/csrc/wg_obs.h

```cpp
#pragma once
#include "wg_device.h"

#define WG_OBSV(v, mn, rng) (raw ? (v) : wg_clip1(wg_scale((v), (mn), (rng))))
template <int L>
__device__ inline float wg_group_sum(float s) {
#pragma unroll
    for (int o = 1; o < L; o <<= 1) s += __shfl_xor(s, o, 64);
    return s;
}
template <int L>
__device__ inline float wg_ring_sum_g(const WgRing& r, const int lo, const int hi, const int sub) {
    constexpr int U = L == 1 ? 8 : 4;
    float s = 0.f;
#pragma nounroll
    for (int q = lo + sub; q < hi; q += U * L) {
        float v[U];
#pragma unroll
        for (int k = 0; k < U; ++k) v[k] = r.at(min(q + k * L, hi - 1));
#pragma unroll
        for (int k = 0; k < U; ++k)
            if (q + k * L < hi) s += v[k];
    }
    return wg_group_sum<L>(s);
}
template <int L>
__device__ inline float wg_calc_ti_g(const WgRing& r, const int sub) {
    constexpr int U = L == 1 ? 8 : 4;
    const int avail = r.avail();
    const float U_ = wg_ring_sum_g<L>(r, 0, avail, sub) / (float)avail;
    float m2 = 0.f;
#pragma nounroll
    for (int q = sub; q < avail; q += U * L) {
        float v[U];
#pragma unroll
        for (int k = 0; k < U; ++k) v[k] = r.at(min(q + k * L, avail - 1));
#pragma unroll
        for (int k = 0; k < U; ++k)
            if (q + k * L < avail) { const float dv = v[k] - U_; m2 += dv * dv; }
    }
    m2 = wg_group_sum<L>(m2);
    return sqrtf(m2 / (float)avail) / U_;
}

template <int L>
__device__ inline void build_obs(const WgParams& p, const WgPtrs& d, int ctx_id, int lane, float* __restrict__ obs,
                                 float* __restrict__ obs2, const float* rbase, const float* fbase,
                                 const bool raw = false, float* __restrict__ obs_m = nullptr,
                                 const int n_pushed_known = -1, float* mscratch = nullptr) {
    const int N = p.N;
    const int n_pushed = n_pushed_known >= 0 ? n_pushed_known : d.ctx[ctx_id].n_pushed;
    float ti_sum = 0.f;
    float buf[8];
    const int sub = lane & (L - 1), per_pass = WG_WAVE / L;
    const bool wr = sub == 0;
    int n_turb_vals = 0;
    for (int t = lane / L; t < N; t += per_pass) {
        float* o = obs + (size_t)t * p.turb_obs;
        int n = 0;
        for (int ch = 0; ch < WG_N_CH; ++ch) {
            const int H = p.ch[ch].history_len;
            if (ch == WG_CH_POWER && p.turb_ti) {
                WgRing r(rbase + p.ring_off[WG_CH_WS] + t, n_pushed, p.ch[WG_CH_WS].history_len, N, p.ring_cap[WG_CH_WS]);
                float v = WG_OBSV(wg_calc_ti_g<L>(r, sub), p.ti_min_f, p.ti_rng_f);
                if (wr) {
                    o[n] = v; if (obs2) obs2[(size_t)t * p.turb_obs + n] = v;
                    if (obs_m) obs_m[(size_t)t * p.obs_dim_multi + n] = v;
                }
                ++n;
            }
            WgRing r(rbase + p.ring_off[ch] + t, n_pushed, H, N, p.ring_cap[ch]);
            const bool on = p.turb_on[ch] != 0;
            const bool cur_on = p.ch[ch].current && on, rol_on = p.ch[ch].rolling_mean && on;
            const int avail = r.avail();
            if (avail == 0) continue;
            if (cur_on) {
                float v = WG_OBSV(r.at(avail - 1), p.sc_min[ch], p.sc_rng[ch]);
                if (wr) {
                    o[n] = v; if (obs2) obs2[(size_t)t * p.turb_obs + n] = v;
                    if (obs_m) obs_m[(size_t)t * p.obs_dim_multi + n] = v;
                }
                ++n;
            }
            if (rol_on) {
                const int W = p.ch[ch].window_len, HN = p.ch[ch].history_n;
                for (int i = 0; i < HN; ++i) {
                    int lo, hi;
                    if (i == 0) { lo = avail - W; if (lo < 0) lo = 0; hi = avail; }
                    else if (i == HN - 1 && avail >= W) { lo = 0; hi = W; }
                    else if (avail < W) { lo = 0; hi = avail; }
                    else {
                        int spacing = (avail - W) / (HN - 1); if (spacing < 1) spacing = 1;
                        int pos = i * spacing; if (pos > avail - W) pos = avail - W;
                        lo = pos; hi = pos + W;
                    }
                    const float s = wg_ring_sum_g<L>(r, lo, hi, sub);
                    float v = WG_OBSV(s / (float)(hi - lo), p.sc_min[ch], p.sc_rng[ch]);
                    if (wr) {
                        o[n] = v; if (obs2) obs2[(size_t)t * p.turb_obs + n] = v;
                        if (obs_m) obs_m[(size_t)t * p.obs_dim_multi + n] = v;
                    }
                    ++n;
                }
            }
        }
        n_turb_vals = n;
        if (p.farm_ti) {
            WgRing r(rbase + p.ring_off[WG_CH_WS] + t, n_pushed, p.ch[WG_CH_WS].history_len, N, p.ring_cap[WG_CH_WS]);
            const float ti = wg_calc_ti_g<L>(r, sub);
            if (wr) ti_sum += raw ? ti : wg_scale(ti, p.ti_min_f, p.ti_rng_f);
        }
    }
    if (obs_m) {
        const int nt = __shfl(n_turb_vals, 0, 64);
        int m = 0;
        if (lane == 0) m = wg_turb_block_b(p, rbase, fbase, n_pushed, 0, true, mscratch);
        m = __shfl(m, 0, 64);
        asm volatile("s_waitcnt vmcnt(0) lgkmcnt(0)" ::: "memory");
        for (int i = lane; i < N * m; i += WG_WAVE) {
            const int t = i / m, k = i - t * m;
            obs_m[(size_t)t * p.obs_dim_multi + nt + k] = wg_clip1(mscratch[k]);
        }
    }
    if (p.farm_ti) ti_sum = wg_wave_sum(ti_sum);
    if (lane == 0 && p.farm_obs > 0) {
        float* o = obs + (size_t)N * p.turb_obs;
        float* o2 = obs2 ? obs2 + (size_t)N * p.turb_obs : nullptr;
        int n = 0;
        const int chs[3] = {WG_CH_WS, WG_CH_WD, WG_CH_POWER};
        for (int ci = 0; ci < 3; ++ci) {
            const int ch = chs[ci];
            if (ch == WG_CH_POWER && p.farm_ti) {
                float v = raw ? ti_sum / (float)N : wg_clip1(ti_sum / (float)N);
                o[n] = v; if (o2) o2[n] = v;
                ++n;
            }
            if (!p.farm_on[ch]) continue;
            WgRing r(fbase + p.fring_off[ch], n_pushed, p.ch[ch].history_len, 1, p.ring_cap[ch]);
            const float rng = ch == WG_CH_POWER ? p.sc_rng_farm_power : p.sc_rng[ch];
            const int cnt = (p.ch[ch].current ? 1 : 0) + (p.ch[ch].rolling_mean ? p.ch[ch].history_n : 0);
            if (cnt <= 8 && !raw) {
                int m = wg_mes_get(p.ch[ch], p.ch[ch].current, p.ch[ch].rolling_mean, r, p.sc_min[ch], rng, buf);
                for (int i = 0; i < m; ++i) { float v = wg_clip1(buf[i]); o[n] = v; if (o2) o2[n] = v; ++n; }
            } else {
                const int avail = r.avail();
                if (avail == 0) continue;
                if (p.ch[ch].current) { float v = WG_OBSV(r.at(avail - 1), p.sc_min[ch], rng); o[n] = v; if (o2) o2[n] = v; ++n; }
                if (p.ch[ch].rolling_mean) {
                    const int W = p.ch[ch].window_len, HN = p.ch[ch].history_n;
                    for (int i = 0; i < HN; ++i) {
                        int lo, hi;
                        if (i == 0) { lo = avail - W; if (lo < 0) lo = 0; hi = avail; }
                        else if (i == HN - 1 && avail >= W) { lo = 0; hi = W; }
                        else if (avail < W) { lo = 0; hi = avail; }
                        else {
                            int spacing = (avail - W) / (HN - 1); if (spacing < 1) spacing = 1;
                            int pos = i * spacing; if (pos > avail - W) pos = avail - W;
                            lo = pos; hi = pos + W;
                        }
                        const float s = wg_ring_sum(r, lo, hi);
                        float v = WG_OBSV(s / (float)(hi - lo), p.sc_min[ch], rng);
                        o[n] = v; if (o2) o2[n] = v; ++n;
                    }
                }
            }
        }
    }
}

struct ObsIn {
    double S[WG_N_SUMS];
    float cur[WG_N_CH];
};
struct SumsRaw {
    double S[WG_N_SUMS];
    float nw[WG_N_CH];
    float lv[WG_N_SUMS];
};
__device__ __forceinline__ int wg_umod(int n, int H, unsigned magic) {
    if (H == 1) return 0;
    int r = n - (int)__umulhi((unsigned)n, magic) * H;
    if (r >= H) r -= H;
    if (r < 0) r += H;
    return r;
}
struct SumsEnt {
    const float* rb; int stride; bool farm; unsigned sm, cm;
};
template <bool TURB = false>
__device__ __forceinline__ SumsEnt wg_sums_ent(const WgParams& p, const WgPtrs& d, const int ctx_id, const int ent) {
    SumsEnt q;
    q.farm = TURB ? false : ent == p.N;
    q.rb = q.farm ? d.fring + (size_t)ctx_id * p.fring_stride : d.ring + (size_t)ctx_id * p.ring_stride + ent;
    q.stride = q.farm ? 1 : p.N;
    q.sm = q.farm ? p.sum_mask_f : p.sum_mask_t;
    q.cm = q.farm ? p.cur_mask_f : p.cur_mask_t;
    return q;
}
template <bool GEN, bool NEWEST = true, bool TURB = false>
__device__ inline SumsRaw wg_sums_load(const WgParams& p, const WgPtrs& d, const int e, const int ctx_id, const int ent, const int np) {
    constexpr int NSL = GEN ? WG_N_SUMS : WG_N_CH;
    SumsRaw r;
    const SumsEnt q = wg_sums_ent<TURB>(p, d, ctx_id, ent);
    const int NS = p.N + 1;
    const double* ws_ = d.wsum + (size_t)ctx_id * WG_N_SUMS * NS + ent;
    const unsigned ti = GEN ? q.sm >> WG_SUM_TI1 : 0u;
#pragma unroll
    for (int ch = 0; ch < WG_N_CH; ++ch) {
        const bool need = (((q.sm | q.cm) >> ch) & 1u) || (ch == WG_CH_WS && ti);
        const int off = q.farm ? p.fring_off[ch] : p.ring_off[ch];
        r.nw[ch] = (NEWEST && need) ? q.rb[off + wg_umod(np, p.ring_cap[ch], p.ring_magic[ch]) * q.stride] : 0.f;
    }
#pragma unroll
    for (int s = 0; s < WG_N_SUMS; ++s) { r.S[s] = 0.0; r.lv[s] = 0.f; }
#pragma unroll
    for (int s = 0; s < NSL; ++s) {
        if ((q.sm >> s) & 1u) {
            const int ch = s < WG_N_CH ? s : WG_CH_WS;
            const int off = q.farm ? p.fring_off[ch] : p.ring_off[ch];
            const int Wc = p.sum_w[s];
            r.S[s] = ws_[(size_t)s * NS];
            if (np >= Wc) r.lv[s] = q.rb[off + wg_umod(np - Wc, p.ring_cap[ch], p.ring_magic[ch]) * q.stride];
        }
    }
    return r;
}
template <bool GEN>
__device__ inline ObsIn wg_sums_apply(const WgParams& p, const WgPtrs& d, const int ctx_id, const int ent, const SumsRaw& r, const bool store) {
    constexpr int NSL = GEN ? WG_N_SUMS : WG_N_CH;
    ObsIn o;
    const int NS = p.N + 1;
    const unsigned sm = ent == p.N ? p.sum_mask_f : p.sum_mask_t;
    double* ws_ = d.wsum + (size_t)ctx_id * WG_N_SUMS * NS + ent;
#pragma unroll
    for (int s = 0; s < WG_N_SUMS; ++s) o.S[s] = 0.0;
#pragma unroll
    for (int s = 0; s < NSL; ++s) {
        if ((sm >> s) & 1u) {
            const int ch = s < WG_N_CH ? s : WG_CH_WS;
            double v = (double)r.nw[ch], l = (double)r.lv[s];
            if (s == WG_SUM_TI2) { v = v * v; l = l * l; }
            o.S[s] = (r.S[s] - l) + v;
            if (store) ws_[(size_t)s * NS] = o.S[s];
        }
    }
#pragma unroll
    for (int ch = 0; ch < WG_N_CH; ++ch) o.cur[ch] = r.nw[ch];
    return o;
}
__device__ __forceinline__ float wg_scale_r(const float v, const float mn, const float inv_rng) {
    return wg_clip1(2.0f * (v - mn) * inv_rng - 1.0f);
}
template <typename OC>
__device__ __forceinline__ float wg_sums_mean(const OC& oc, const double S, const int ch, const int n_pushed) {
    const int H = oc.hlen[ch], W = oc.wlen[ch];
    const int wc = W < H ? W : H;
    if (n_pushed >= wc) return (float)(S * oc.inv_w[ch]);
    return (float)(S / (double)n_pushed);
}
template <typename OC>
__device__ __forceinline__ float wg_sums_ti(const OC& oc, const double S1, const double S2, const int n_pushed) {
    const int H = oc.hlen[WG_CH_WS];
    const double n = (double)(n_pushed < H ? n_pushed : H);
    const double U = S1 / n;
    double var = S2 / n - U * U;
    if (!(var > 0.0)) var = 0.0;
    return (float)(sqrt(var) / U);
}
template <bool GEN, typename OC>
__device__ __forceinline__ int wg_obs_turbine(const OC& oc, const double* S, const float* cur, const int n_pushed,
                                              float* __restrict__ o, float* __restrict__ o2, float* __restrict__ om,
                                              float* __restrict__ om2 = nullptr) {
    int n = 0;
#define WG_EMIT(v_) do { const float _v = (v_); o[n] = _v; if (o2) o2[n] = _v; if (om) om[n] = _v; if (om2) om2[n] = _v; ++n; } while (0)
#pragma unroll
    for (int ch = 0; ch < WG_N_CH; ++ch) {
        if (GEN && ch == WG_CH_POWER && oc.turb_ti)
            WG_EMIT(wg_scale_r(wg_sums_ti(oc, S[WG_SUM_TI1], S[WG_SUM_TI2], n_pushed), oc.ti_mn, oc.inv_ti_rng));
        if (n_pushed == 0) continue;
        if ((oc.cur_mask >> ch) & 1u) WG_EMIT(wg_scale_r(cur[ch], oc.mn[ch], oc.inv_rng[ch]));
        if ((oc.rol_mask >> ch) & 1u) WG_EMIT(wg_scale_r(wg_sums_mean(oc, S[ch], ch, n_pushed), oc.mn[ch], oc.inv_rng[ch]));
    }
#undef WG_EMIT
    return n;
}

template <bool MULTI, bool GEN, typename Get>
__device__ inline void build_obs_sums(const WgParams& p, const int lane, float* __restrict__ obs, float* __restrict__ obs2,
                                      float* __restrict__ obs_m, const int n_pushed, float* mscratch, const ObsIn& first, Get get,
                                      float* __restrict__ obs_m2 = nullptr) {
    const int N = p.N;
    float ti_sum = 0.f;
    int n_turb_vals = 0;
    for (int t = lane; t < N; t += WG_WAVE) {
        const ObsIn oi = t == lane ? first : get(t);
        n_turb_vals = wg_obs_turbine<GEN>(p.oc, oi.S, oi.cur, n_pushed, obs + (size_t)t * p.turb_obs,
                                          obs2 ? obs2 + (size_t)t * p.turb_obs : nullptr,
                                          (MULTI && obs_m) ? obs_m + (size_t)t * p.obs_dim_multi : nullptr,
                                          (MULTI && obs_m2) ? obs_m2 + (size_t)t * p.obs_dim_multi : nullptr);
        if (GEN && p.farm_ti) ti_sum += 2.0f * (wg_sums_ti(p.oc, oi.S[WG_SUM_TI1], oi.S[WG_SUM_TI2], n_pushed) - p.oc.ti_mn) * p.oc.inv_ti_rng - 1.0f;
    }
    if (!GEN) return;
    const bool farm_any = p.farm_obs > 0 || (MULTI && obs_m != nullptr);
    if (!farm_any) return;
    if (p.farm_ti) ti_sum = wg_wave_sum(ti_sum);
    ObsIn of{};
    if (lane == 0 && (p.sum_mask_f | p.cur_mask_f)) of = get(N);
    if (MULTI && obs_m) {
        const int nt = __shfl(n_turb_vals, 0, 64);
        int m = 0;
        if (lane == 0) {
#pragma unroll
            for (int ch = 0; ch < WG_N_CH; ++ch) {
                if (ch == WG_CH_POWER && p.farm_ti)
                    mscratch[m++] = wg_scale_r(wg_sums_ti(p.oc, of.S[WG_SUM_TI1], of.S[WG_SUM_TI2], n_pushed), p.oc.ti_mn, p.oc.inv_ti_rng);
                if (ch == WG_CH_YAW || !p.farm_on[ch] || n_pushed == 0) continue;
                const float irng = ch == WG_CH_POWER ? 1.0f / p.sc_rng_farm_power : p.oc.inv_rng[ch];
                if (p.ch[ch].current) mscratch[m++] = wg_scale_r(of.cur[ch], p.oc.mn[ch], irng);
                if (p.ch[ch].rolling_mean) mscratch[m++] = wg_scale_r(wg_sums_mean(p.oc, of.S[ch], ch, n_pushed), p.oc.mn[ch], irng);
            }
        }
        m = __shfl(m, 0, 64);
        asm volatile("s_waitcnt vmcnt(0) lgkmcnt(0)" ::: "memory");
        for (int i = lane; i < N * m; i += WG_WAVE) {
            const int t = i / m, k = i - t * m;
            obs_m[(size_t)t * p.obs_dim_multi + nt + k] = mscratch[k];
            if (obs_m2) obs_m2[(size_t)t * p.obs_dim_multi + nt + k] = mscratch[k];
        }
    }
    if (lane == 0 && p.farm_obs > 0) {
        float* o = obs + (size_t)N * p.turb_obs;
        float* o2 = obs2 ? obs2 + (size_t)N * p.turb_obs : nullptr;
        int n = 0;
        const int chs[3] = {WG_CH_WS, WG_CH_WD, WG_CH_POWER};
#pragma unroll
        for (int ci = 0; ci < 3; ++ci) {
            const int ch = chs[ci];
            if (ch == WG_CH_POWER && p.farm_ti) { const float v = wg_clip1(ti_sum / (float)N); o[n] = v; if (o2) o2[n] = v; ++n; }
            if (!p.farm_on[ch] || n_pushed == 0) continue;
            const float irng = ch == WG_CH_POWER ? 1.0f / p.sc_rng_farm_power : p.oc.inv_rng[ch];
            if (p.ch[ch].current) { const float v = wg_scale_r(of.cur[ch], p.oc.mn[ch], irng); o[n] = v; if (o2) o2[n] = v; ++n; }
            if (p.ch[ch].rolling_mean) {
                const float v = wg_scale_r(wg_sums_mean(p.oc, of.S[ch], ch, n_pushed), p.oc.mn[ch], irng);
                o[n] = v; if (o2) o2[n] = v; ++n;
            }
        }
    }
}
```

### windgym_amd/csrc/wg_plan.h

```cpp
#pragma once
#include <algorithm>
#include <cmath>
#include <cstring>
#include <string>
#include <vector>

#ifndef __HIPCC__
struct float4;
#endif
#include "wg_flow.h"

struct WgHookInt {
    bool set = false;
    int v = 0;
};
struct WgHooks {
    WgHookInt flow_block, flow_res, flow_env, env_wpe, env_split, step_fused, sums, lds_pad, lf_cap, pstride_pad, step_graph, share_dev;
    bool first_obs_gl_only = false, no_box8 = false, debug = false, timeline = false;
    std::string timeline_out;
};

struct WgPlan {
    WgParams p;
    FlowP f;
    int envw_eligible;
    int fused_eligible;
    int first_obs;
    double tab_x0, tab_dx;
    int reset_chunk, reset_launches;
    double alg_bytes;
};

inline double wg_defd(double v, double dflt) { return v == 0.0 ? dflt : v; }

inline int wg_plan_fail(std::string* err, int code, const std::string& msg) {
    if (err) *err = msg;
    return code;
}

inline int wg_validate_config(const wg_config* c, std::string* err) {
    if (!c) return wg_plan_fail(err, WG_ERR_INVALID, "null argument");
    if (c->abi_version != WG_ABI_VERSION) return wg_plan_fail(err, WG_ERR_INVALID, "abi_version mismatch");
    if (c->n_envs < 1 || c->n_turb < 1) return wg_plan_fail(err, WG_ERR_INVALID, "n_envs and n_turb must be >= 1");
    if (c->n_farms != 1 && c->n_farms != 2) return wg_plan_fail(err, WG_ERR_INVALID, "n_farms must be 1 or 2");
    if (c->k_sub < 1) return wg_plan_fail(err, WG_ERR_INVALID, "dt_env must be a multiple of dt_sim");
    if (c->n_particles < 8 || c->n_particles % 4) return wg_plan_fail(err, WG_ERR_INVALID, "n_particles must be a multiple of 4 (>= 8)");
    if (c->n_rotor_pts < 1 || c->n_rotor_pts > 64) return wg_plan_fail(err, WG_ERR_INVALID, "n_rotor_pts must be in [1, 64]");
    if (c->n_turb > 32 * WG_MASK_WORDS) return wg_plan_fail(err, WG_ERR_UNSUPPORTED, "n_turb > 128 is not supported by this build");
    if ((long long)c->n_turb * c->n_particles >= (1ll << 22) || c->n_particles > 16384)
        return wg_plan_fail(err, WG_ERR_UNSUPPORTED, "n_turb * n_particles must stay below 2^22 (and n_particles <= 16384)");
    if (!c->x_pos || !c->y_pos || !c->rotor_dy || !c->rotor_dz || !c->tab_ws || !c->tab_power || !c->tab_ct || c->n_tab < 2)
        return wg_plan_fail(err, WG_ERR_INVALID, "layout / rotor points / turbine table missing");
    if (c->action_method != WG_ACT_YAW && c->action_method != WG_ACT_WIND)
        return wg_plan_fail(err, WG_ERR_UNSUPPORTED, "The ActionMethod must be yaw or wind (absolute is not implemented)");
    if (c->reward_mode < 0 || c->reward_mode > 3)
        return wg_plan_fail(err, WG_ERR_INVALID, "The Power_reward must be either Baseline, Power_avg, None or Power_diff");
    if (c->reward_mode == WG_REW_POWER_DIFF && c->power_avg < 40)
        return wg_plan_fail(err, WG_ERR_INVALID, "The Power_avg must be larger then 40 for the Power_diff reward");
    if (c->reward_mode == WG_REW_BASELINE && c->n_farms != 2)
        return wg_plan_fail(err, WG_ERR_INVALID, "Baseline reward needs the baseline farm (n_farms = 2)");
    if (c->power_avg < 1) return wg_plan_fail(err, WG_ERR_INVALID, "Power_avg must be >= 1");
    if (c->turb_mode < WG_TURB_NONE || c->turb_mode > WG_TURB_BOX_POOL) return wg_plan_fail(err, WG_ERR_INVALID, "Invalid turbulence type specified");
    for (int i = 0; i < WG_N_CH; ++i)
        if (c->ch[i].history_len < 1 || c->ch[i].window_len < 1 || c->ch[i].history_n < 1)
            return wg_plan_fail(err, WG_ERR_INVALID, "sensor history/window lengths must be >= 1");
    {
        const double ka = wg_defd(c->m0_ka, 0.38), kb = wg_defd(c->m0_kb, 0.004), hill = wg_defd(c->m0_hill, 0.4);
        const double tia = c->no_ti_fold ? 0.0 : 0.466 * wg_defd(c->m0_ti_a, 0.73);
        const double k_hi = ka * std::sqrt(c->ti_max * c->ti_max + tia * tia) + kb;
        if (k_hi > 0.25 || std::fabs(hill) * c->ws_max > 16.0)
            return wg_plan_fail(err, WG_ERR_INVALID, "wind ranges exceed the 16-bit emission record: need ka*sqrt(TI_max^2 + 0.34^2) + kb <= 0.25 "
                                                     "(TI_max <= 0.55 with the default constants) and |hill| * ws_max <= 16 m/s");
    }
    if (c->deficit_model < 0 || c->deficit_model > 2)
        return wg_plan_fail(err, WG_ERR_INVALID, "deficit_model must be 0 (Gaussian), 1 (super-Gaussian) or 2 (tabulated eddy-viscosity deficit)");
    return 0;
}

inline int wg_plan_ch_count(const wg_channel& c, int on) { return (c.current && on) + (c.rolling_mean && on) * c.history_n; }

inline void wg_plan_scalars(const wg_config* c, WgParams& p) {
    p.B = c->n_envs; p.N = c->n_turb; p.F = c->n_farms; p.K = c->k_sub; p.P = c->n_particles; p.S = c->n_rotor_pts;
    p.NP = p.N * p.P;
    p.dt = (float)c->dt_sim; p.dt_d = c->dt_sim;
    p.D = (float)c->rotor_diameter; p.D_d = c->rotor_diameter; p.inv_D = 1.0f / (float)c->rotor_diameter;
    p.hub = (float)c->hub_height; p.hub_d = c->hub_height;
    p.dpart = c->d_particle * c->rotor_diameter;
    p.yaw_min = (float)c->yaw_min; p.yaw_max = (float)c->yaw_max; p.yaw_step = (float)c->yaw_step;
    p.yaw_min_d = c->yaw_min; p.yaw_max_d = c->yaw_max; p.yaw_step_d = c->yaw_step; p.yaw_start = c->yaw_start;
    p.action_method = c->action_method; p.base_controller = c->base_controller; p.yaw_init = c->yaw_init;
    p.has_yaw_defined = c->yaw_defined != nullptr;
    p.ws_min = c->ws_min; p.ws_max = c->ws_max; p.ti_min = c->ti_min; p.ti_max = c->ti_max;
    p.wd_min = c->wd_min; p.wd_max = c->wd_max; p.n_passthrough = c->n_passthrough;
    p.never_truncate = c->never_truncate;
    p.full_chains = c->full_chains;
    for (int i = 0; i < WG_N_CH; ++i) p.ch[i] = c->ch[i];
    p.turb_on[WG_CH_WS] = c->turb_ws; p.turb_on[WG_CH_WD] = c->turb_wd; p.turb_on[WG_CH_YAW] = 1;
    p.turb_on[WG_CH_POWER] = c->turb_power;
    p.farm_on[WG_CH_WS] = c->farm_ws; p.farm_on[WG_CH_WD] = c->farm_wd; p.farm_on[WG_CH_YAW] = 0;
    p.farm_on[WG_CH_POWER] = c->farm_power;
    p.turb_ti = c->turb_ti; p.farm_ti = c->farm_ti;
    const double mn[WG_N_CH] = {c->ws_scale_min, c->wd_scale_min, c->yaw_min, 0.0};
    const double mx[WG_N_CH] = {c->ws_scale_max, c->wd_scale_max, c->yaw_max, c->power_max};
    for (int i = 0; i < WG_N_CH; ++i) { p.sc_min[i] = (float)mn[i]; p.sc_rng[i] = (float)(mx[i] - mn[i]); }
    p.sc_rng_farm_power = (float)(c->power_max * c->n_turb);
    p.ti_min_f = (float)c->ti_scale_min; p.ti_rng_f = (float)(c->ti_scale_max - c->ti_scale_min);
    p.noise = c->noise;
    for (int i = 0; i < WG_N_CH; ++i) p.noise_sigma[i] = (float)c->noise_sigma[i];
    p.reward_mode = c->reward_mode; p.power_avg = c->power_avg; p.power_scaling = c->power_scaling;
    p.action_penalty = c->action_penalty; p.penalty_type = c->penalty_type;
    p.fill_a = c->fill_steps_agent; p.fill_b = c->fill_steps_base; p.autoreset = c->autoreset;
    p.extra_inc = c->extra_timestep_inc; p.turb_mode = c->turb_mode;
    p.ka = (float)wg_defd(c->m0_ka, 0.38); p.kb = (float)wg_defd(c->m0_kb, 0.004); p.eps0 = (float)wg_defd(c->m0_eps, 0.2);
    p.hill = (float)wg_defd(c->m0_hill, 0.4);
    p.tia = (float)wg_defd(c->m0_ti_a, 0.73); p.tib = (float)wg_defd(c->m0_ti_b, 0.8325);
    p.tic = (float)wg_defd(c->m0_ti_c, 0.0325); p.tid = (float)wg_defd(c->m0_ti_d, -0.32);
    p.fc_scale = wg_defd(c->m0_fc_scale, 2.0);
    p.n_tab = c->n_tab;
    double sx = 0, sy = 0;
    for (int t = 0; t < p.N; ++t) { sx += c->x_pos[t]; sy += c->y_pos[t]; }
    p.cx0 = sx / p.N; p.cy0 = sy / p.N;
}

inline void wg_plan_obs_layout(const wg_config* c, WgParams& p) {
    p.turb_obs = wg_plan_ch_count(c->ch[WG_CH_WS], c->turb_ws) + wg_plan_ch_count(c->ch[WG_CH_WD], c->turb_wd) +
                 wg_plan_ch_count(c->ch[WG_CH_YAW], 1) + (c->turb_ti ? 1 : 0) + wg_plan_ch_count(c->ch[WG_CH_POWER], c->turb_power);
    p.farm_obs = wg_plan_ch_count(c->ch[WG_CH_WS], c->farm_ws) + wg_plan_ch_count(c->ch[WG_CH_WD], c->farm_wd) +
                 (c->farm_ti ? 1 : 0) + wg_plan_ch_count(c->ch[WG_CH_POWER], c->farm_power);
    p.obs_dim = p.turb_obs * p.N + p.farm_obs;
    p.obs_dim_multi = p.turb_obs + p.farm_obs;
    p.hist_max = std::max(c->ch[WG_CH_WS].history_len, std::max(c->ch[WG_CH_WD].history_len, c->ch[WG_CH_YAW].history_len));
    for (int i = 0; i < WG_N_CH; ++i) {
        const bool on = p.turb_on[i] != 0;
        int st = 0;
        if (on && c->ch[i].current) st = 1;
        if (on && c->ch[i].rolling_mean) st = 2;
        if (i == WG_CH_WS && (c->turb_ti || c->farm_ti)) st = 2;
        p.stage_ch[i] = st;
    }
}

inline void wg_plan_sums(const wg_config* c, const WgHooks& hk, WgParams& p) {
    bool ok = true;
    for (int i = 0; i < WG_N_CH; ++i) {
        const bool used = p.turb_on[i] || (i != WG_CH_YAW && p.farm_on[i]);
        if (used && c->ch[i].rolling_mean && c->ch[i].history_n != 1) ok = false;
    }
    if (hk.sums.set && hk.sums.v == 0) ok = false;
    p.sums_mode = ok ? 1 : 0;
    for (int i = 0; i < WG_N_CH; ++i) {
        p.ring_cap[i] = c->ch[i].history_len + (ok ? 1 : 0);
        p.ring_magic[i] = (unsigned)((1ull << 32) / (unsigned long long)p.ring_cap[i]) + 1u;
    }
    if (ok) {
        for (int i = 0; i < WG_N_CH; ++i) {
            p.sum_w[i] = std::min(c->ch[i].window_len, c->ch[i].history_len);
            if (p.turb_on[i] && c->ch[i].rolling_mean) p.sum_mask_t |= 1u << i;
            if (p.turb_on[i] && c->ch[i].current) p.cur_mask_t |= 1u << i;
            if (i != WG_CH_YAW && p.farm_on[i] && c->ch[i].rolling_mean) p.sum_mask_f |= 1u << i;
            if (i != WG_CH_YAW && p.farm_on[i] && c->ch[i].current) p.cur_mask_f |= 1u << i;
        }
        p.sum_w[WG_SUM_TI1] = p.sum_w[WG_SUM_TI2] = c->ch[WG_CH_WS].history_len;
        if (c->turb_ti || c->farm_ti) p.sum_mask_t |= (1u << WG_SUM_TI1) | (1u << WG_SUM_TI2);
        if (c->farm_ti) p.sum_mask_f |= (1u << WG_SUM_TI1) | (1u << WG_SUM_TI2);
    }
    WgObsCfg& oc = p.oc;
    oc.cur_mask = p.cur_mask_t; oc.rol_mask = p.sum_mask_t & 0xfu;
    oc.turb_ti = c->turb_ti; oc.turb_obs = p.turb_obs; oc.obs_dim = p.obs_dim; oc.obs_dim_multi = p.obs_dim_multi;
    for (int i = 0; i < WG_N_CH; ++i) {
        oc.hlen[i] = c->ch[i].history_len; oc.wlen[i] = c->ch[i].window_len;
        oc.mn[i] = p.sc_min[i]; oc.inv_rng[i] = 1.0f / p.sc_rng[i];
        oc.inv_w[i] = 1.0 / (double)std::min(c->ch[i].window_len, c->ch[i].history_len);
    }
    oc.ti_mn = p.ti_min_f; oc.inv_ti_rng = 1.0f / p.ti_rng_f;
    int off = 0, foff = 0;
    for (int i = 0; i < WG_N_CH; ++i) {
        p.ring_off[i] = off; off += p.N * p.ring_cap[i];
        p.fring_off[i] = foff; foff += p.ring_cap[i];
    }
    p.ring_stride = off; p.fring_stride = foff;
}

inline int wg_plan_pstride(int NP, const WgHooks& hk) {
    size_t pstride = ((size_t)NP + 63) / 64;
    if (pstride % 2 == 0) pstride += 1;
    pstride *= 64;
    if (hk.pstride_pad.set) pstride = (size_t)NP + (size_t)hk.pstride_pad.v;
    return (int)pstride;
}

inline bool wg_uniform_grid(const wg_config* c, int* n, double* x0, double* dx) {
    bool uniform = true;
    const double dx0 = c->tab_ws[1] - c->tab_ws[0];
    for (int i = 2; i < c->n_tab; ++i)
        if (std::fabs((c->tab_ws[i] - c->tab_ws[i - 1]) - dx0) > 1e-9 * std::fabs(dx0)) uniform = false;
    *n = uniform ? c->n_tab : 1024;
    *x0 = c->tab_ws[0];
    *dx = uniform ? dx0 : (c->tab_ws[c->n_tab - 1] - c->tab_ws[0]) / (*n - 1);
    return uniform;
}
inline void wg_uniform_table(const wg_config* c, std::vector<float>* power, std::vector<float>* ct, double* x0, double* dx) {
    int nu = 0;
    const bool uniform = wg_uniform_grid(c, &nu, x0, dx);
    power->clear(); ct->clear();
    if (uniform) {
        for (int i = 0; i < nu; ++i) { power->push_back((float)c->tab_power[i]); ct->push_back((float)c->tab_ct[i]); }
        return;
    }
    int k = 0;
    for (int i = 0; i < nu; ++i) {
        const double x = std::min(*x0 + i * *dx, c->tab_ws[c->n_tab - 1]);
        while (k + 2 < c->n_tab && c->tab_ws[k + 1] <= x) ++k;
        const double f = (x - c->tab_ws[k]) / (c->tab_ws[k + 1] - c->tab_ws[k]);
        power->push_back((float)(c->tab_power[k] + f * (c->tab_power[k + 1] - c->tab_power[k])));
        ct->push_back((float)(c->tab_ct[k] + f * (c->tab_ct[k + 1] - c->tab_ct[k])));
    }
}

struct WgFlowVariant {
    bool small;
    int res, block;
    int tc0;
    int ql_shift, ql_lpt_shift;
};

inline WgFlowVariant wg_plan_flow_variant(const WgParams& p, const WgHooks& hk) {
    WgFlowVariant v;
    int tc = 1024 / p.N; if (tc < 1) tc = 1; if (tc > p.N) tc = p.N;
    v.tc0 = tc;
    v.small = p.N <= 32 && tc == p.N;
    v.res = v.small ? 1 : 0;
    v.block = v.small ? 64 : 256;
    if (!v.small && p.N <= 255 && p.turb_mode == WG_TURB_NONE) v.res = 1;
    if ((hk.flow_block.set && hk.flow_block.v == 256) || (hk.flow_res.set && hk.flow_res.v == 0)) { v.res = 0; v.block = 256; }
    v.ql_shift = 0;
    while ((1 << v.ql_shift) < p.P / 4) ++v.ql_shift;
    if (((long)p.N << v.ql_shift) > 65536) { v.res = 0; v.block = 256; }
    v.ql_lpt_shift = 0;
    while (v.ql_lpt_shift < 3 && (p.N << (v.ql_lpt_shift + 1)) <= v.block) ++v.ql_lpt_shift;
    return v;
}

struct WgFlowCarve {
    int target_chunk, lf_cap, gl, lds_off_ql, lds_off_gat, lds_off_turb, lds_off_tab;
    size_t bytes;
};

inline WgFlowCarve wg_plan_flow_carve(const WgParams& p, const WgHooks& hk, const WgFlowVariant& v, int res, int block, int n_tab_u, int S_shift,
                                      int added) {
    WgFlowCarve k;
    int tc = v.tc0;
    k.lf_cap = 0; k.gl = 0; k.lds_off_ql = 0; k.lds_off_gat = 0;
    size_t off = sizeof(float) * 4 * (size_t)tc * p.N;
    if (res) {
        const size_t ql = ((size_t)p.NP / 2 + 15) & ~(size_t)15;
        if (!v.small) {
            const size_t budget = std::max(ql, off) + sizeof(float) * (size_t)tc * p.N;
            const int fit = (int)((budget - 16) / (10 * (size_t)p.N));
            tc = std::max(tc, std::min(p.N, fit));
        }
        off = std::max(ql, ((size_t)(added ? 22 : 10) * tc * p.N + 16 + 15) & ~(size_t)15);
        if (block == 256) {
            const size_t fixed = WG_LF_OFF_DEF(p.N);
            off = std::max(off, (fixed + 8 * 512 + 15) & ~(size_t)15);
            k.lf_cap = (int)((off - fixed) / 8);
            if (hk.lf_cap.set) k.lf_cap = std::max(64, std::min(k.lf_cap, hk.lf_cap.v));
        }
        if (block == 64 && p.turb_mode == WG_TURB_NONE) {
            k.gl = 1;
            off = ((size_t)10 * tc * p.N + 16 + 15) & ~(size_t)15;
            k.lds_off_ql = (int)off; off += ql;
            k.lds_off_gat = (int)off; off += WG_GAT_BYTES;
        }
    }
    k.target_chunk = tc;
    k.lds_off_turb = (int)off; off += (size_t)WG_TURB_LDS_BYTES * p.N;
    off = (off + 15) & ~(size_t)15;
    k.lds_off_tab = (int)off;
    off += sizeof(float) * (2 * (size_t)n_tab_u + 2 * (size_t)p.S) + (k.gl ? 0 : sizeof(unsigned) * WG_MASK_WORDS * (size_t)tc) +
           (res ? 0 : sizeof(float) * (size_t)tc * p.N);
    off += sizeof(int) * (4 * (size_t)p.N + 4);
    if (added && res) off += sizeof(float) * 3 * ((size_t)p.N << S_shift) + sizeof(int) * (size_t)tc;
    k.bytes = (off + 15) & ~(size_t)15;
    return k;
}

inline size_t wg_plan_farm_quads(const wg_config* c, const WgParams& p) {
    size_t qf = 0;
    for (int t = 0; t < p.N; ++t) {
        double dm = 0;
        for (int j = 0; j < p.N; ++j) dm = std::max(dm, std::hypot(c->x_pos[j] - c->x_pos[t], c->y_pos[j] - c->y_pos[t]));
        long len = (((long)(dm / p.dpart) + 4) + 3) & ~3L;
        if (len > p.P || p.full_chains) len = p.P;
        qf += (size_t)len / 4;
    }
    return qf;
}

inline bool wg_plan_env(const WgParams& p, FlowP& f, bool small, size_t qf, int lds_limit) {
    const int NSl = 2 * p.F, NL = NSl * p.N;
    const size_t clb = ((size_t)2 * NL * (p.N > 1 ? p.N - 1 : 1) + 15) & ~(size_t)15;
    const size_t stage = std::max((size_t)8 * WG_ENV_CAP + clb, ((size_t)2 * NSl * qf + 15) & ~(size_t)15);
    f.env_off_tab = (int)((WG_ENV_FIXED_LDS_BYTES + stage + 15) & ~(size_t)15);
    const size_t o = (size_t)f.env_off_tab + sizeof(float) * (2 * (size_t)f.n_tab + 2 * (size_t)p.S);
    f.env_lds = (int)((o + 15) & ~(size_t)15);
    return f.res && small && f.block == 64 && f.gl && p.turb_mode == WG_TURB_NONE && NL <= 64 && p.N <= 32 && p.P <= 4096 && !f.added &&
           f.deficit_model == 0 && f.env_lds <= 32768 && f.env_lds <= lds_limit;
}

struct WgEnvbCarve {
    int env_cap, off_cl, off_tab;
    size_t bytes;
};
inline WgEnvbCarve wg_plan_envb_carve(const WgParams& p, int n_tab_u, int wpe) {
    WgEnvbCarve k;
    const int nlp = wpe == 4 ? 16 : 64;
    const int nl_w = (wpe == 4 ? 1 : (wpe == 2 ? p.F : 2 * p.F)) * p.N;
    k.env_cap = wpe == 4 ? 128 : 256;
    size_t ob = WG_ENVB_FIXED_LDS_BYTES(nlp) + (size_t)20 * k.env_cap;
    k.off_cl = (int)ob;
    ob = (ob + (size_t)2 * nl_w * (p.N > 1 ? p.N - 1 : 1) + 15) & ~(size_t)15;
    k.off_tab = (int)ob;
    ob += sizeof(float) * (2 * (size_t)n_tab_u + 2 * (size_t)p.S);
    k.bytes = (ob + 15) & ~(size_t)15;
    return k;
}

inline bool wg_plan_envb(const WgParams& p, const WgHooks& hk, FlowP& f, bool small, int lds_limit, int* wpe) {
    const int NL = 2 * p.F * p.N;
    *wpe = (p.B <= 2048) ? 2 : 1;
    if (hk.env_wpe.set) {
        const int w = hk.env_wpe.v;
        *wpe = (w == 4 && p.F == 2 && p.N <= 16) ? 4 : (w == 2 ? 2 : (w == 4 ? 2 : 1));
    }
    if (!(f.res && small && f.block == 64 && !f.gl && p.turb_mode >= WG_TURB_BOX && NL <= 64 && p.N <= 32 && p.P <= 4096 && f.S_pad <= 16 &&
          f.deficit_model == 0))
        return false;
    WgEnvbCarve k = wg_plan_envb_carve(p, f.n_tab, *wpe);
    while (*wpe > 1 && *wpe * k.bytes + 64 > (size_t)lds_limit) {
        *wpe /= 2;
        k = wg_plan_envb_carve(p, f.n_tab, *wpe);
    }
    f.env_cap = k.env_cap; f.envb_off_cl = k.off_cl; f.env_off_tab = k.off_tab; f.env_lds = (int)k.bytes;
    return f.env_lds <= 32768 && f.env_lds <= lds_limit;
}

inline void wg_plan_step_kernels(const wg_config* c, const WgHooks& hk, const WgParams& p, FlowP& f, bool small, int lds_limit) {
    const size_t qf = wg_plan_farm_quads(c, p);
    const bool env_ok = wg_plan_env(p, f, small, qf, lds_limit);
    int envb_wpe = 1;
    const bool envb_ok = wg_plan_envb(p, hk, f, small, lds_limit, &envb_wpe);
    f.env_inc = 1 + (p.extra_inc ? 1 : 0);
    f.env_eps_max = std::min(1.0f, (float)(p.eps0 * std::sqrt(3.0))) + 2.0f / 65535.0f;
    f.envw = ((env_ok || envb_ok) && !hk.flow_block.set && !hk.flow_res.set) ? 1 : 0;
    if (hk.flow_env.set) f.envw = ((env_ok || envb_ok) && hk.flow_env.v != 0) ? 1 : 0;
    f.env_wpe = (p.B <= 2048 && 2 * f.env_lds <= lds_limit) ? 2 : 1;
    if (hk.env_wpe.set) f.env_wpe = (hk.env_wpe.v == 2 && 2 * f.env_lds <= lds_limit) ? 2 : 1;
    const bool split_ok = env_ok && f.env_wpe == 2 && p.K == 1 && 4 * f.env_lds + 4096 <= lds_limit;
    f.env_split = (split_ok && p.B <= 1024 && qf >= 256) ? (p.B <= 512 ? 2 : 1) : 0;
    if (hk.env_split.set) f.env_split = (hk.env_split.v != 0 && split_ok && p.B <= 2048) ? (hk.env_split.v == 2 ? 2 : 1) : 0;
    if (envb_ok) f.env_wpe = envb_wpe;
    f.env_share = (f.envw && env_ok && p.F == 2) ? 1 : 0;
    if (hk.share_dev.set && hk.share_dev.v == 0) f.env_share = 0;
    const bool gen = p.turb_ti || p.farm_ti || p.farm_obs > 0 || (p.sum_mask_f | p.cur_mask_f) != 0;
    f.env_fused = (f.envw && p.sums_mode && !gen && p.power_avg <= 64) ? 1 : 0;
    if (hk.step_fused.set) f.env_fused = (f.env_fused && hk.step_fused.v != 0) ? 1 : 0;
}

inline void wg_plan_flow_scalars(const wg_config* c, const WgParams& p, double tab_x0, double tab_dx, FlowP& f) {
    f.B = p.B; f.N = p.N; f.F = p.F; f.K = p.K; f.P = p.P; f.S = p.S; f.NP = p.NP;
    f.S_pad = 1; f.S_shift = 0;
    while (f.S_pad < p.S) { f.S_pad <<= 1; f.S_shift++; }
    f.autoreset = p.autoreset; f.action_method = p.action_method; f.base_controller = p.base_controller;
    f.power_avg = p.power_avg; f.script_rows = 0; f.noise = (p.noise == WG_NOISE_NORMAL);
    f.dt = p.dt; f.D = p.D; f.inv_D = p.inv_D; f.hub = p.hub; f.dpart_f = (float)p.dpart; f.R_rot = 0.5f * p.D;
    f.inv_N = 1.0f / (float)p.N; f.inv_S = 1.0f / (float)p.S; f.inv_P = 1.0f / (float)p.P;
    f.inv_power_avg = 1.0f / (float)(p.power_avg > 0 ? p.power_avg : 1);
    f.pavg_magic = (unsigned)((1ull << 32) / (unsigned long long)(p.power_avg > 0 ? p.power_avg : 1)) + 1u;
    f.dt_d = p.dt_d; f.dpart = p.dpart; f.inv_dpart = 1.0 / p.dpart;
    f.yaw_min = p.yaw_min; f.yaw_max = p.yaw_max; f.yaw_step = p.yaw_step;
    f.ka = p.ka; f.kb = p.kb; f.eps0 = p.eps0; f.hill = p.hill; f.tia = p.tia; f.tib = p.tib; f.tic = p.tic; f.tid = p.tid;
    f.tab_x0 = (float)tab_x0; f.tab_inv_dx = (float)(1.0 / tab_dx);
    f.ue_scale = p.turb_mode == WG_TURB_NONE ? 1.0f : 2.0f;
    for (int i = 0; i < WG_N_CH; ++i) {
        f.hlen[i] = p.ring_cap[i]; f.ring_off[i] = p.ring_off[i]; f.fring_off[i] = p.fring_off[i];
        f.inv_hlen[i] = 1.0f / (float)p.ring_cap[i];
        f.hmagic[i] = (unsigned)((1ull << 32) / (unsigned long long)p.ring_cap[i]) + 1u;
        f.noise_sigma[i] = p.noise_sigma[i];
    }
    f.ring_stride = p.ring_stride; f.fring_stride = p.fring_stride;
    f.turb_mode = p.turb_mode; f.fc_scale = p.fc_scale; f.D_d = p.D_d; f.hub_d = p.hub_d;
    f.inv_sqrt_S = 1.0f / std::sqrt((float)p.S);
    f.added = (c->added_turbulence != 0 && c->turb_mode != WG_TURB_NONE) ? 1 : 0;
    f.no_ti_fold = c->no_ti_fold != 0; f.deficit_model = c->deficit_model;
    f.km1 = (float)wg_defd(c->m0_km1, 0.6); f.km2r = (float)(2.0 * wg_defd(c->m0_km2, 0.35) * 0.5 * p.D_d);
    f.sg_af = (float)wg_defd(c->m0_sg_af, 3.11); f.sg_bf = (float)wg_defd(c->m0_sg_bf, -0.68); f.sg_cf = (float)wg_defd(c->m0_sg_cf, 2.41);
    f.an_inv_ka = (float)(1.0 / wg_defd(c->m0_ka, 0.38));
}

inline int wg_plan_reset_launches(const wg_config* c, const WgParams& p, int reset_chunk) {
    double xmn = 1e300, xmx = -1e300, ymn = 1e300, ymx = -1e300;
    for (int t = 0; t < p.N; ++t) {
        xmn = std::min(xmn, c->x_pos[t]); xmx = std::max(xmx, c->x_pos[t]);
        ymn = std::min(ymn, c->y_pos[t]); ymx = std::max(ymx, c->y_pos[t]);
    }
    const double ext_x = xmx - xmn, ext_y = ymx - ymn;
    const double diag = std::sqrt(ext_x * ext_x + ext_y * ext_y);
    const double ws_lo = std::max(1e-3, std::min(c->ws_min, c->ws_max));
    const long max_dev = (long)std::ceil(2.0 * diag / ws_lo / c->dt_sim) + 2;
    const long max_work = max_dev + (long)p.K * (std::max(p.fill_a, p.fill_b) + 1);
    return (int)((max_work + reset_chunk - 1) / reset_chunk) + 1;
}

inline double wg_plan_alg_bytes(const WgParams& p) {
    const bool turb = p.turb_mode != WG_TURB_NONE, boxm = p.turb_mode >= WG_TURB_BOX;
    const double per_farm_step = (double)p.NP * (4 + 4 + 8 + (turb ? 24 : 0) + (boxm ? 64 : 0)) +
                                 (double)p.N * (7 * 4 * 2 + 16) + (boxm ? (double)p.N * p.S * 96 : 0.0);
    return (double)p.B * ((double)p.K * p.F * per_farm_step + 20.0 * p.N + 12.0 * p.obs_dim + 20.0);
}

inline int wg_plan_create(const wg_config* c, const WgHooks& hk, int lds_limit, WgPlan* out, std::string* err) {
    memset(out, 0, sizeof(*out));
    WgParams& p = out->p;
    FlowP& f = out->f;
    wg_plan_scalars(c, p);
    wg_plan_obs_layout(c, p);
    wg_plan_sums(c, hk, p);
    wg_uniform_grid(c, &f.n_tab, &out->tab_x0, &out->tab_dx);
    wg_plan_flow_scalars(c, p, out->tab_x0, out->tab_dx, f);
    f.pstride = wg_plan_pstride(p.NP, hk);

    const WgFlowVariant v = wg_plan_flow_variant(p, hk);
    f.res = v.res; f.block = v.block; f.ql_shift = v.ql_shift; f.ql_lpt_shift = v.ql_lpt_shift;
    WgFlowCarve k = wg_plan_flow_carve(p, hk, v, f.res, f.block, f.n_tab, f.S_shift, f.added);
    if (f.res && k.bytes > (size_t)lds_limit) {
        f.res = 0; f.block = 256;
        k = wg_plan_flow_carve(p, hk, v, f.res, f.block, f.n_tab, f.S_shift, f.added);
    }
    if (k.bytes > (size_t)lds_limit)
        return wg_plan_fail(err, WG_ERR_UNSUPPORTED, "wg_create: k_flow needs " + std::to_string(k.bytes) + " bytes of LDS per workgroup (limit " +
                                                     std::to_string(lds_limit) + "): too many turbines for one workgroup");
    if (f.deficit_model != 0 && !f.res)
        return wg_plan_fail(err, WG_ERR_UNSUPPORTED, "deficit_model 1 / 2 (super-Gaussian, eddy-viscosity table) are built into the compact k_flow variants only "
                                                     "(farms of up to 32 turbines, larger ones with steady inflow)");
    p.compact = f.res;
    f.target_chunk = k.target_chunk; f.lf_cap = k.lf_cap; f.gl = k.gl; f.lds_off_ql = k.lds_off_ql; f.lds_off_gat = k.lds_off_gat;
    f.lds_off_turb = k.lds_off_turb; f.lds_off_tab = k.lds_off_tab;
    f.lds_bytes = (int)k.bytes;
    if (hk.lds_pad.set) f.lds_bytes = std::min(lds_limit, f.lds_bytes + hk.lds_pad.v);
    f.rec_il = (f.res && p.turb_mode == WG_TURB_NONE) ? 1 : 0;

    wg_plan_step_kernels(c, hk, p, f, v.small, lds_limit);
    out->envw_eligible = f.envw; out->fused_eligible = f.env_fused;
    out->first_obs = (f.gl || (f.res && p.sums_mode && !hk.first_obs_gl_only)) ? 1 : 0;
    out->reset_chunk = 32;
    out->reset_launches = wg_plan_reset_launches(c, p, out->reset_chunk);
    out->alg_bytes = wg_plan_alg_bytes(p);
    return 0;
}

inline void wg_plan_step_path(const WgPlan& plan, long long box_cells, long long abox_cells, int* envw, int* env_fused) {
    const bool big = plan.f.turb_mode != WG_TURB_NONE && (box_cells >= (1ll << 28) || abox_cells >= (1ll << 28));
    *envw = (plan.envw_eligible && !big) ? 1 : 0;
    *env_fused = (plan.fused_eligible && *envw) ? 1 : 0;
}
```

Before: 92.43 million.

## Pack hot env-kernel parameters into contiguous kernarg groups for scalar loads

Adds a compact 'hot' parameter block after the shared kernel arguments, grouped by kernel phase (prologue, setup, early request, tail, farm), so each phase loads its fields with a few wide scalar loads instead of scattered reads through the cold argument structure. It also loads four adjacent context words as one int4 and generalises the sums and lean-early helpers to take these compact structs. The goal is less scalar memory latency and fewer SGPR-heavy pointer chases in the prologue, at the cost of a larger kernarg segment and duplicated parameter copies that must stay in sync with the host plan.

```diff
diff --git a/windgym_amd/csrc/wg_env.hip b/windgym_amd/csrc/wg_env.hip
--- a/windgym_amd/csrc/wg_env.hip
+++ b/windgym_amd/csrc/wg_env.hip
@@ -5,6 +5,37 @@
 #endif
 #include "wg_env_common.h"
 #include "wg_internal.h"
+#include "wg_plan.h"
+
+struct EnvKArgsHot { EnvKArgs a; EnvHotP hot; };
+static_assert(offsetof(EnvKArgsHot, hot) == sizeof(EnvKArgs) && sizeof(EnvKArgs) % alignof(EnvHotP) == 0,
+              "the hot block follows the shared arguments without a gap (the kernarg segment lays it out by the same rule)");
+typedef const __attribute__((address_space(4))) EnvHotP* EnvHotPtr;
+__device__ __forceinline__ EnvHotPtr wg_hot_args() {
+    const __attribute__((address_space(4))) EnvKArgsHot* k = (const __attribute__((address_space(4))) EnvKArgsHot*)__builtin_amdgcn_kernarg_segment_ptr();
+    asm volatile("" : "+s"(k));
+    return &k->hot;
+}
+__device__ __forceinline__ EnvHotFarm env_farm_cold() {
+    const KArgsPtr k = wg_cold_args();
+    EnvHotFarm m;
+    m.fring = k->d.fring; m.step_farm_pow = k->d.step_farm_pow; m.step_base_pow = k->d.step_base_pow; m.pend_farm = k->d.pend_farm;
+    m.pend_base = k->d.pend_base; m.fring_stride = k->p.fring_stride; m.power_avg = k->p.power_avg; m.pavg_magic = k->p.pavg_magic;
+    m.inv_N = k->p.inv_N;
+#pragma unroll
+    for (int i = 0; i < WG_N_CH; ++i) { m.hlen[i] = k->p.hlen[i]; m.fring_off[i] = k->p.fring_off[i]; m.hmagic[i] = k->p.hmagic[i]; }
+    return m;
+}
+__device__ __forceinline__ EnvHotTail env_tail_cold() {
+    const KArgsPtr k = wg_cold_args();
+    EnvHotTail m;
+    m.ring = k->d.ring; m.cur_ws = k->d.cur_ws; m.cur_wd = k->d.cur_wd; m.env = k->d.env;
+    m.n_tab = k->p.n_tab; m.tab_x0 = k->p.tab_x0; m.tab_inv_dx = k->p.tab_inv_dx; m.env_off_tab = k->p.env_off_tab; m.ring_stride = k->p.ring_stride;
+#pragma unroll
+    for (int i = 0; i < WG_N_CH; ++i) { m.hlen[i] = k->p.hlen[i]; m.ring_off[i] = k->p.ring_off[i]; m.inv_hlen[i] = k->p.inv_hlen[i]; m.noise_sigma[i] = k->p.noise_sigma[i]; }
+    return m;
+}
+#define WG_HOT(group) (*(const decltype(EnvHotP::group)*)&wg_hot_args()->group)
 
 struct __attribute__((aligned(16))) EnvSlotLds {
     int dev_rem, fill_rem, sub, budget;
@@ -96,13 +127,10 @@
 __device__ __forceinline__ void env_flow(char* const smem, char* const smem_pass, float* const zone, const int wv, const int role, const int mode,
                                          const float* __restrict__ actions, const uint8_t* __restrict__ mask, const int chunk, EnvFlowOut& out) {
     const int tid = threadIdx.x & 63, e = blockIdx.x;
-    int N, F, NS, NL;
-    float inv_N;
-    {
-        const KArgsPtr ka = wg_cold_args();
-        N = ka->p.N; F = ka->p.F; inv_N = ka->p.inv_N;
-        NS = WPE == 2 ? F : 2 * F; NL = NS * N;
-    }
+    const EnvHotPro hp = WG_HOT(pro);
+    const int N = hp.N, F = hp.F;
+    const float inv_N = hp.inv_N;
+    const int NS = WPE == 2 ? F : 2 * F, NL = NS * N;
     const int kbase = WPE == 2 ? wv * F : 0;
     const bool valid = tid < NL;
     const int g = valid ? tid : 0;
@@ -129,13 +157,11 @@
     bool parked = false;
     float yaw, tu, tti, oyaw;
     {
-        const KArgsPtr k0 = wg_cold_args();
         static_assert(sizeof(WgEnv) == 128, "the env header is loaded as 32 words");
-        const int hw = reinterpret_cast<const int*>(k0->d.env + e)[tid & 31];
-        if (GLUE != 0 && tid < 32) reinterpret_cast<int*>(smem + WG_ENV_OFF_HDR)[tid] = hw;
+        const int hw = reinterpret_cast<const int*>(hp.env + e)[tid & 31];
         out.bg_init_pending = 0; out.rounds = 0; out.first_obs = 0;
         const bool use_mask = mode == WG_MODE_RESET && mask != nullptr;
-        const uint8_t mask_byte = *(use_mask ? mask + e : reinterpret_cast<const uint8_t*>(k0->d.env + e));
+        const uint8_t mask_byte = *(use_mask ? mask + e : reinterpret_cast<const uint8_t*>(hp.env + e));
         const bool masked_out = use_mask && mask_byte == 0;
         const unsigned ctx_id = (unsigned)(e * 2 + c), slot_id = (unsigned)(e * 2 * F + kbase + k);
         const unsigned tb = (unsigned)((e * 2 * F + kbase) * N + g);
@@ -147,30 +173,32 @@
         float ti_f, wd_env, l_yaw, l_u, l_ti, l_act;
         float4 l_bnd;
         int l_roff, l_rnext;
-        auto load_state = [&]() __attribute__((always_inline)) {
-            const KArgsPtr kl = wg_cold_args();
-            const WgSlot& slot = kl->d.slot[slot_id];
-            const WgCtx& cx = kl->d.ctx[ctx_id];
+        auto load_state = [&](const EnvHotPro& kl) __attribute__((always_inline)) {
+            const WgSlot& slot = kl.slot[slot_id];
+            const WgCtx& cx = kl.ctx[ctx_id];
             dev_rem = slot.dev_remaining; fill_rem = slot.fill_remaining;
             s_off = slot.s_off; c_time = slot.time; c_head = slot.head; n_valid = slot.n_valid; c_istep = slot.istep;
             n_emitted = slot.n_emitted; c_part = slot.part_count; c_flow = slot.flow_count; c_add = slot.add_count;
             ws = cx.ws; ti_f = (float)cx.ti; wd_env = (float)cx.wd;
-            n_pushed = cx.n_pushed; pend_farm_n = cx.pend_farm_n; pend_base_n = cx.pend_base_n;
-            c_tag = (unsigned)cx.episode_tag; init_pending = cx.init_pending; time_max_c = cx.time_max;
-            const int* ro = kl->d.roff + ctx_id * (unsigned)(N + 1);
+            n_pushed = cx.n_pushed; time_max_c = cx.time_max;
+            static_assert(offsetof(WgCtx, episode_tag) == 80 && offsetof(WgCtx, pend_farm_n) == 84 && offsetof(WgCtx, pend_base_n) == 88 &&
+                          offsetof(WgCtx, init_pending) == 92 && alignof(WgCtx) >= 16, "the context's words 80 .. 95 are loaded as one int4");
+            const int4 cw = *reinterpret_cast<const int4*>(&cx.episode_tag);
+            c_tag = (unsigned)cw.x; pend_farm_n = cw.y; pend_base_n = cw.z; init_pending = cw.w;
+            const int* ro = kl.roff + ctx_id * (unsigned)(N + 1);
             l_roff = ro[(unsigned)t]; l_rnext = ro[(unsigned)t + 1u];
-            l_xr = kl->d.xr[tcx]; l_yr = kl->d.yr[tcx];
-            l_yaw = kl->d.yaw[tb]; l_u = kl->d.u[tb]; l_ti = kl->d.ti_loc[tb];
-            l_bnd = reinterpret_cast<const float4*>(kl->d.bnd)[tb];
+            l_xr = kl.xr[tcx]; l_yr = kl.yr[tcx];
+            l_yaw = kl.yaw[tb]; l_u = kl.u[tb]; l_ti = kl.ti_loc[tb];
+            l_bnd = reinterpret_cast<const float4*>(kl.bnd)[tb];
         };
-        load_state();
-        const int n_tab = k0->p.n_tab, S = k0->p.S;
+        load_state(hp);
+        const int n_tab = hp.n_tab, S = hp.S;
         const unsigned i_tab = (unsigned)min(tid, n_tab - 1), i_s = (unsigned)min(tid, S - 1);
-        const float pf_tp = k0->d.tab_power[i_tab], pf_tc = k0->d.tab_ct[i_tab];
-        const float pf_dy = k0->d.rotor_dy[i_s], pf_dz = k0->d.rotor_dz[i_s];
+        const float pf_tp = hp.tab_power[i_tab], pf_tc = hp.tab_ct[i_tab];
+        const float pf_dy = hp.rotor_dy[i_s], pf_dz = hp.rotor_dz[i_s];
         {
             const bool has_act = mode == WG_MODE_STEP && farm == 0;
-            const float a = *(has_act ? actions + (unsigned)(e * N + t) : k0->d.tab_ct);
+            const float a = *(has_act ? actions + (unsigned)(e * N + t) : hp.tab_ct);
             l_act = has_act ? a : 0.f;
         }
 
@@ -179,6 +207,7 @@
         int env_done = WG_HDR_I(done), env_shadow_iters = WG_HDR_I(shadow_iters), env_steps_done = WG_HDR_I(steps_done);
         int env_timestep = WG_HDR_I(timestep), env_time_max_live = WG_HDR_I(time_max_live);
 #undef WG_HDR_I
+        if (GLUE != 0 && tid < 32) reinterpret_cast<int*>(smem + WG_ENV_OFF_HDR)[tid] = hw;
         if (SPLIT && role == 1) {
             if (tid == 0) { *reinterpret_cast<int*>(smem + WG_ENV_OFF_HDR) = 0; if (GLUE != 0 && (SPLIT == 1 || wv == 0)) reinterpret_cast<int*>(zone)[LEAN_PRE_FLAG] = 0; }
             asm volatile("s_waitcnt vmcnt(0) lgkmcnt(0)" ::: "memory");
@@ -188,8 +217,8 @@
             asm volatile("s_barrier" ::: "memory");
         }
         if (SPLIT && role == 1 && GLUE != 0 && c == env_live) {
-            const EnvKArgsPtr kz = (EnvKArgsPtr)wg_cold_args();
-            const LeanEarly zr = lean_early_load(*(const WgParams*)&kz->gp, *(const WgPtrs*)&kz->gd, e, N, F, tid, hw);
+            const EnvHotReq kz = WG_HOT(req);
+            const LeanEarly zr = lean_early_load(kz, e, N, F, tid, hw);
             double* const zs = reinterpret_cast<double*>(zone);
 #pragma unroll
             for (int sI = 0; sI < WG_N_CH; ++sI) { zs[LEAN_PRE_S(sI, tid)] = zr.S[sI]; zone[LEAN_PRE_LV(sI, tid)] = zr.lv[sI]; }
@@ -203,7 +232,7 @@
         out.steps_done = env_steps_done; out.time_max_live = env_time_max_live;
 
         const bool is_live_c = (c == env_live);
-        const int autoreset = k0->p.autoreset;
+        const int autoreset = hp.autoreset;
         int budget = 0;
         long plan_left = 0;
         if (mode == WG_MODE_STEP) {
@@ -220,7 +249,10 @@
                 const WgParams& gp = *ki->d.gp;
                 env_init_episode<GLUE != 0>(e, env_live ^ 1, tid);
                 full_barrier<64>();
-                load_state();
+                {
+                    const EnvHotPro hr = WG_HOT(pro);
+                    load_state(hr);
+                }
                 const int fill_max = F == 2 ? max(gp.fill_a, gp.fill_b) : gp.fill_a;
                 const int tm = WPE == 2 ? ki->d.ctx[e * 2 + env_live].time_max : __shfl(time_max_c, env_live * F * N, 64);
                 const long total = wg_rule_episode_steps(tm, gp.extra_inc);
@@ -229,28 +261,29 @@
                 budget = wg_shadow_share(dev_rem + gp.K * fill_rem, total - env_steps_done, env_steps_done, e, farm ? 0x80000000u : 0u);
                 plan_left = total - env_steps_done;
             } else {
-                const long total = wg_rule_episode_steps_inc(env_time_max_live, k0->p.env_inc);
-                budget = role_dev ? wg_shadow_share(dev_rem + k0->p.K * fill_rem, total - env_steps_done, env_steps_done, e, farm ? 0x80000000u : 0u) : 0;
+                const long total = wg_rule_episode_steps_inc(env_time_max_live, hp.env_inc);
+                budget = role_dev ? wg_shadow_share(dev_rem + hp.K * fill_rem, total - env_steps_done, env_steps_done, e, farm ? 0x80000000u : 0u) : 0;
                 plan_left = total - env_steps_done;
             }
         } else {
             role_dev = is_live_c && !masked_out;
             budget = chunk;
+            asm volatile("" : : "v"(init_pending));
         }
         bool clone_here = false;
-        if (k0->p.env_share) {
+        if (hp.env_share) {
             const int dev_a = __shfl(dev_rem, (tid - N) & 63, 64);
             parked = valid && role_dev && farm == 1 && dev_rem > 0 && c_istep == 0u && dev_a > 0;
             const int twin_fill = __shfl(parked ? fill_rem + 1 : 0, (tid + N) & 63, 64);
             const bool lead = valid && role_dev && farm == 0 && twin_fill > 0;
             if (lead && mode == WG_MODE_STEP && !defer_init)
-                budget = wg_shadow_share(dev_rem + k0->p.K * max(fill_rem, twin_fill - 1), plan_left, env_steps_done, e);
+                budget = wg_shadow_share(dev_rem + hp.K * max(fill_rem, twin_fill - 1), plan_left, env_steps_done, e);
             if (parked) budget = 0;
             clone_here = lead && budget >= dev_rem;
         }
         if (SPLIT) {
             const bool two = valid && role_dev && budget >= 2;
-            split_on = mode == WG_MODE_STEP && k0->p.K == 1 && (is_live_c || (SPLIT == 2 && !out.bg_init_pending)) && !defer_init && !__ballot(two) &&
+            split_on = mode == WG_MODE_STEP && hp.K == 1 && (is_live_c || (SPLIT == 2 && !out.bg_init_pending)) && !defer_init && !__ballot(two) &&
                        !__ballot(clone_here);
             if (role == 1 && !split_on) return;
         }
@@ -272,7 +305,7 @@
             }
         }
 
-        const KArgsPtr k1 = wg_cold_args();
+        const EnvHotSet k1 = WG_HOT(set);
         const int rlen = l_rnext - l_roff;
         const int head = n_emitted == 0u ? rlen - 1 : fast_mod((int)(n_emitted - 1u), rlen, __builtin_amdgcn_rcpf((float)rlen));
         const float ws_f = (float)ws;
@@ -285,29 +318,29 @@
             if (t == 0) {
                 my.dev_rem = dev_rem; my.fill_rem = fill_rem; my.sub = 0; my.budget = budget;
                 my.n_valid = n_valid; my.n_emitted = n_emitted; my.n_emitted0 = n_emitted;
-                my.move_max = fabsf(k1->p.hill) * ws_f * k1->p.dt; my.ti_pow = fast_pow(ti_f, k1->p.tic);
+                my.move_max = fabsf(k1.hill) * ws_f * k1.dt; my.ti_pow = fast_pow(ti_f, k1.tic);
                 my.s_off = s_off; my.ws = ws; my.ws_f = ws_f; my.ti_f = ti_f; my.wd_env = wd_env; my.base_acc = 0.f;
                 my.n_pushed = n_pushed; my.pend_farm_n = pend_farm_n; my.pend_base_n = pend_base_n; my.n_flow = 0;
                 my.bg_init = out.bg_init_pending;
                 my.c_time = c_time; my.c_head = c_head; my.c_part = c_part; my.c_flow = c_flow; my.c_istep = c_istep; my.c_tag = c_tag; my.c_add = c_add;
             }
         }
-        float* const tabp = reinterpret_cast<float*>(smem + k1->p.env_off_tab);
+        float* const tabp = reinterpret_cast<float*>(smem + k1.env_off_tab);
         float* const tabct = tabp + n_tab;
         float2* const rpt = reinterpret_cast<float2*>(tabct + n_tab);
-        const float hub = k1->p.hub;
+        const float hub = k1.hub;
         auto rp = [&](const float dy_, const float dz_) __attribute__((always_inline)) {
             const float dz = hub + dz_ - hub;
             return make_float2(dy_, dz * dz);
         };
         if (tid < n_tab) { tabp[tid] = pf_tp; tabct[tid] = pf_tc; }
         if (tid < S) rpt[tid] = rp(pf_dy, pf_dz);
-        for (int i = tid + 64; i < n_tab; i += 64) { tabp[i] = k1->d.tab_power[i]; tabct[i] = k1->d.tab_ct[i]; }
-        for (int i = tid + 64; i < S; i += 64) rpt[i] = rp(k1->d.rotor_dy[i], k1->d.rotor_dz[i]);
+        for (int i = tid + 64; i < n_tab; i += 64) { tabp[i] = k1.tab_power[i]; tabct[i] = k1.tab_ct[i]; }
+        for (int i = tid + 64; i < S; i += 64) rpt[i] = rp(k1.rotor_dy[i], k1.rotor_dz[i]);
 
         yaw = l_yaw; tu = l_u; tti = l_ti; oyaw = l_yaw;
         if (role_live && farm == 0 && valid) {
-            yaw = wg_rule_adjust_yaw(k1->p.action_method, yaw, l_act, k1->p.yaw_min, k1->p.yaw_max, k1->p.yaw_step);
+            yaw = wg_rule_adjust_yaw(k1.action_method, yaw, l_act, k1.yaw_min, k1.yaw_max, k1.yaw_step);
         }
     }
     float tpow = 0.f, tct = 0.f, cg = 1.f;
@@ -322,9 +355,9 @@
             if (WPE == 2 && wv != env_live) {
                 out.g_early = LeanEarly{};
             } else {
-                const EnvKArgsPtr kz = (EnvKArgsPtr)wg_cold_args();
+                const EnvHotReq kz = WG_HOT(req);
                 const int hwl = reinterpret_cast<const int*>(smem + WG_ENV_OFF_HDR)[tid & 31];
-                out.g_early = lean_early_load(*(const WgParams*)&kz->gp, *(const WgPtrs*)&kz->gd, e, N, F, tid, hwl);
+                out.g_early = lean_early_load(kz, e, N, F, tid, hwl);
             }
         }
     };
@@ -739,7 +772,7 @@
 
         const bool measuring = stepping && !is_dev;
         const bool unit_end = measuring && (sub + 1 == K);
-        const KArgsPtr kc = wg_cold_args();
+        const EnvHotTail kc = WPE == 2 ? env_tail_cold() : WG_HOT(tail);
         const float inv_k = 1.0f / (float)K;
         const unsigned ctx_id = (unsigned)(e * 2 + c);
         if (stepping) {
@@ -752,9 +785,9 @@
                 part_acc += min(my.new_valid, rg.y);
             }
             stepped = true;
-            const int n_tab = kc->p.n_tab;
-            const float tab_x0 = kc->p.tab_x0, tab_inv_dx = kc->p.tab_inv_dx;
-            const float* const tabp = reinterpret_cast<const float*>(smem + kc->p.env_off_tab);
+            const int n_tab = kc.n_tab;
+            const float tab_x0 = kc.tab_x0, tab_inv_dx = kc.tab_inv_dx;
+            const float* const tabp = reinterpret_cast<const float*>(smem + kc.env_off_tab);
             const float wsn = fmaxf(tu * cg, 0.0f);
             tpow = env_tab(tabp, tab_x0, tab_inv_dx, n_tab, wsn);
             tct = env_tab(tabp + n_tab, tab_x0, tab_inv_dx, n_tab, wsn) * cg * cg;
@@ -765,26 +798,26 @@
                 if (unit_end) {
                     const int n_pushed = my.n_pushed;
                     const unsigned tcx = ctx_id * (unsigned)N + (unsigned)t;
-                    kc->d.cur_ws[tcx] = wsm;
-                    kc->d.cur_wd[tcx] = wdm;
+                    kc.cur_ws[tcx] = wsm;
+                    kc.cur_wd[tcx] = wdm;
                     if (K != 1) {
 #pragma unroll
                         for (int ch = 0; ch < WG_N_CH; ++ch) val[ch] *= inv_k;
                     }
                     if (NOISE) {
-                        const uint64_t noise_key = ((CEnvPtr)(kc->d.env + e))->noise_key;
+                        const uint64_t noise_key = ((CEnvPtr)(kc.env + e))->noise_key;
                         const uint32_t episode_tag = my.c_tag;
 #pragma unroll
                         for (int ch = 0; ch < WG_N_CH; ++ch)
-                            if (kc->p.noise_sigma[ch] != 0.f)
-                                val[ch] += kc->p.noise_sigma[ch] * wg_noise_normal(noise_key, (uint32_t)n_pushed, (uint32_t)t,
+                            if (kc.noise_sigma[ch] != 0.f)
+                                val[ch] += kc.noise_sigma[ch] * wg_noise_normal(noise_key, (uint32_t)n_pushed, (uint32_t)t,
                                                                                    (uint32_t)ch, episode_tag);
                     }
-                    float* __restrict__ rbase = kc->d.ring + (size_t)ctx_id * kc->p.ring_stride;
+                    float* __restrict__ rbase = kc.ring + (size_t)ctx_id * kc.ring_stride;
 #pragma unroll
                     for (int ch = 0; ch < WG_N_CH; ++ch) {
-                        const int H = kc->p.hlen[ch];
-                        rbase[(unsigned)(kc->p.ring_off[ch] + fast_mod(n_pushed, H, kc->p.inv_hlen[ch]) * N + t)] = val[ch];
+                        const int H = kc.hlen[ch];
+                        rbase[(unsigned)(kc.ring_off[ch] + fast_mod(n_pushed, H, kc.inv_hlen[ch]) * N + t)] = val[ch];
                     }
                     if (GLUE != 0) {
 #pragma unroll
@@ -809,27 +842,27 @@
             float base_acc = my.base_acc;
             if (measuring && farm == 1) base_acc += a_pw;
             if (unit_end) {
-                const FlowP __attribute__((address_space(4)))& pc = kc->p;
+                const EnvHotFarm pc = WPE == 2 ? env_farm_cold() : WG_HOT(farm);
                 if (farm == 0) {
                     const int n_pushed = my.n_pushed, pend_farm_n = my.pend_farm_n;
-                    float* fbase = kc->d.fring + (size_t)ctx_id * pc.fring_stride;
+                    float* fbase = pc.fring + (size_t)ctx_id * pc.fring_stride;
                     fbase[pc.fring_off[WG_CH_WS] + umod_small(n_pushed, pc.hlen[WG_CH_WS], pc.hmagic[WG_CH_WS])] = a_ws * pc.inv_N;
                     fbase[pc.fring_off[WG_CH_WD] + umod_small(n_pushed, pc.hlen[WG_CH_WD], pc.hmagic[WG_CH_WD])] = a_wd * pc.inv_N;
                     fbase[pc.fring_off[WG_CH_POWER] + umod_small(n_pushed, pc.hlen[WG_CH_POWER], pc.hmagic[WG_CH_POWER])] = a_pw;
                     my.out_pw = a_pw;
-                    if (role_live) kc->d.step_farm_pow[e] = a_pw;
+                    if (role_live) pc.step_farm_pow[e] = a_pw;
                     else {
-                        kc->d.pend_farm[(size_t)ctx_id * pc.power_avg + umod_small(pend_farm_n, pc.power_avg, pc.pavg_magic)] = a_pw;
+                        pc.pend_farm[(size_t)ctx_id * pc.power_avg + umod_small(pend_farm_n, pc.power_avg, pc.pavg_magic)] = a_pw;
                         my.pend_farm_n = pend_farm_n + 1;
                     }
                     my.n_pushed = n_pushed + 1;
                 } else {
                     const float bp = K == 1 ? base_acc : base_acc * inv_k;
                     my.out_pw = bp;
-                    if (role_live) kc->d.step_base_pow[e] = bp;
+                    if (role_live) pc.step_base_pow[e] = bp;
                     else {
                         const int pend_base_n = my.pend_base_n;
-                        kc->d.pend_base[(size_t)ctx_id * pc.power_avg + umod_small(pend_base_n, pc.power_avg, pc.pavg_magic)] = bp;
+                        pc.pend_base[(size_t)ctx_id * pc.power_avg + umod_small(pend_base_n, pc.power_avg, pc.pavg_magic)] = bp;
                         my.pend_base_n = pend_base_n + 1;
                     }
                     base_acc = 0.f;
@@ -916,7 +949,7 @@
 k_flow_env(const FlowP p_, const FlowPtrs d_, const int mode, const float* __restrict__ actions,
            const uint8_t* __restrict__ mask, const int chunk, const WgParams gp_, const WgPtrs gd_,
            float* __restrict__ obs_out, float* __restrict__ reward_out, uint8_t* __restrict__ trunc_out,
-           float* __restrict__ final_obs_out) {
+           float* __restrict__ final_obs_out, const EnvHotP hot_) {
     extern __shared__ __attribute__((aligned(16))) char smem[];
 #ifdef WG_TIMELINE
     if (threadIdx.x == 0) { for (int i = 0; i < 20; ++i) wg_stamps[i] = 0; wg_stamps[14] = wall_clock64(); for (int i = 0; i < 8; ++i) wg_counts[i] = 0; }
@@ -1008,8 +1041,9 @@
 #endif
 }
 
+typedef void (*EnvHotKernel)(FlowP, FlowPtrs, int, const float*, const uint8_t*, int, WgParams, WgPtrs, float*, float*, uint8_t*, float*, EnvHotP);
 template <bool NZ, int G>
-static EnvKernel env_kernel(const int wpe, const int split) {
+static EnvHotKernel env_kernel(const int wpe, const int split) {
     if constexpr (G != 0) {
         if (split == 2) return k_flow_env<NZ, G, 2, 2>;
         if (split == 1) return k_flow_env<NZ, G, 2, 1>;
@@ -1022,10 +1056,11 @@
     const int wpe = p->env_wpe == 2 ? 2 : 1;
     const int split = glue != 0 && wpe == 2 && (p->env_split == 1 || p->env_split == 2) ? p->env_split : 0;
     const size_t lds = (size_t)p->env_lds * (wpe + split) + (split ? LEAN_PRE_BYTES : 0);
-    const EnvKernel k = glue == 2 ? (p->noise ? env_kernel<true, 2>(wpe, split) : env_kernel<false, 2>(wpe, split))
+    const EnvHotP hot = wg_plan_env_hot(*p, *d, *gp, *gd);
+    const EnvHotKernel k = glue == 2 ? (p->noise ? env_kernel<true, 2>(wpe, split) : env_kernel<false, 2>(wpe, split))
                       : glue == 1 ? (p->noise ? env_kernel<true, 1>(wpe, split) : env_kernel<false, 1>(wpe, split))
                                   : (p->noise ? env_kernel<true, 0>(wpe, split) : env_kernel<false, 0>(wpe, split));
-    hipLaunchKernelGGL(k, dim3(p->B), dim3(64 * (wpe + split)), lds, st, *p, *d, mode, actions, mask, chunk, *gp, *gd, obs, reward, trunc, final_obs);
+    hipLaunchKernelGGL(k, dim3(p->B), dim3(64 * (wpe + split)), lds, st, *p, *d, mode, actions, mask, chunk, *gp, *gd, obs, reward, trunc, final_obs, hot);
 }
 
 extern "C" void wg_launch_flow_env(const FlowP* p, const FlowPtrs* d, int mode, const float* actions, const uint8_t* mask,
diff --git a/windgym_amd/csrc/wg_flow.h b/windgym_amd/csrc/wg_flow.h
--- a/windgym_amd/csrc/wg_flow.h
+++ b/windgym_amd/csrc/wg_flow.h
@@ -94,6 +94,54 @@
     WgEnv* env_rw;
 };
 
+struct __attribute__((aligned(16))) EnvHotPro {
+    const WgEnv* env; WgSlot* slot; WgCtx* ctx; const int* roff;
+    const double *xr, *yr; float *yaw, *u;
+    float *ti_loc, *bnd; const float *tab_power, *tab_ct;
+    const float *rotor_dy, *rotor_dz;
+    int N, F; float inv_N; int autoreset;
+    int K, n_tab, S, env_inc;
+    int env_share, pad_[3];
+};
+struct __attribute__((aligned(16))) EnvHotSet {
+    const float *tab_power, *tab_ct, *rotor_dy, *rotor_dz;
+    int env_off_tab, action_method; float yaw_min, yaw_max;
+    float yaw_step, hill, dt, tic;
+    float hub; int pad_[3];
+};
+struct __attribute__((aligned(16))) EnvHotReq {
+    double* wsum; float *ring, *farm_pow, *base_pow;
+    float* metrics; int N, power_avg;
+    int ring_stride; unsigned sum_mask_t, cur_mask_t; int pad_;
+    int ring_off[WG_N_CH], sum_w[WG_N_CH], ring_cap[WG_N_CH];
+    unsigned ring_magic[WG_N_CH];
+};
+struct __attribute__((aligned(16))) EnvHotTail {
+    float *ring, *cur_ws, *cur_wd; const WgEnv* env;
+    int n_tab; float tab_x0, tab_inv_dx; int env_off_tab;
+    int ring_stride, pad_[3];
+    int hlen[WG_N_CH], ring_off[WG_N_CH];
+    float inv_hlen[WG_N_CH], noise_sigma[WG_N_CH];
+};
+struct __attribute__((aligned(16))) EnvHotFarm {
+    float *fring, *step_farm_pow, *step_base_pow, *pend_farm;
+    float* pend_base; int fring_stride, power_avg;
+    unsigned pavg_magic; float inv_N; int pad_[2];
+    int hlen[WG_N_CH], fring_off[WG_N_CH];
+    unsigned hmagic[WG_N_CH];
+};
+struct __attribute__((aligned(16))) EnvHotP {
+    EnvHotPro pro;
+    EnvHotSet set;
+    EnvHotReq req;
+    EnvHotTail tail;
+    EnvHotFarm farm;
+};
+#define WG_ENV_HOT_BYTES (160 + 80 + 128 + 128 + 112)
+static_assert(sizeof(EnvHotPro) == 160 && sizeof(EnvHotSet) == 80 && sizeof(EnvHotReq) == 128 && sizeof(EnvHotTail) == 128 &&
+              sizeof(EnvHotFarm) == 112, "EnvHotP: group sizes");
+static_assert(sizeof(EnvHotP) == WG_ENV_HOT_BYTES, "EnvHotP: no padding between the groups");
+
 #define WG_ENV_SLOT_LDS_BYTES 160
 #define WG_ENV_FIXED_LDS_BYTES (3 * 64 * 16 + 2 * 64 * 8 + 4 * WG_ENV_SLOT_LDS_BYTES + 128)
 #define WG_ENV_CAP 256
diff --git a/windgym_amd/csrc/wg_glue_lean.h b/windgym_amd/csrc/wg_glue_lean.h
--- a/windgym_amd/csrc/wg_glue_lean.h
+++ b/windgym_amd/csrc/wg_glue_lean.h
@@ -257,19 +257,19 @@
     double S[WG_N_CH];
     float lv[WG_N_CH], f_old, b_old, met;
 };
-__device__ __forceinline__ LeanEarly lean_early_load(const WgParams& p, const WgPtrs& d, const int e, const int N, const int F,
-                                                     const int lane, const int hw) {
+template <typename H>
+__device__ __forceinline__ LeanEarly lean_early_load(const H& h, const int e, const int N, const int F, const int lane, const int hw) {
 #define WG_HDR_Z(f) __builtin_amdgcn_readlane(hw, (int)(offsetof(WgEnv, f) / 4))
     const int z_live = WG_HDR_Z(live), z_np = WG_HDR_Z(n_pushed_live), z_fn = WG_HDR_Z(farm_pow_n), z_bn = WG_HDR_Z(base_pow_n);
 #undef WG_HDR_Z
-    const int PA = p.power_avg;
-    const SumsRaw zr = wg_sums_load<false, false, true>(p, d, e, e * 2 + z_live, lane < N ? lane : 0, z_np);
+    const int PA = h.power_avg;
+    const SumsRaw zr = wg_sums_load<false, false, true>(h, h, e, e * 2 + z_live, lane < N ? lane : 0, z_np);
     LeanEarly q;
 #pragma unroll
     for (int s = 0; s < WG_N_CH; ++s) { q.S[s] = zr.S[s]; q.lv[s] = zr.lv[s]; }
-    q.f_old = d.farm_pow[(size_t)e * PA + z_fn % PA];
-    q.b_old = F == 2 ? d.base_pow[(size_t)e * PA + z_bn % PA] : 0.f;
-    q.met = lane < WG_N_METRICS ? d.metrics[(size_t)e * WG_N_METRICS + lane] : 0.f;
+    q.f_old = h.farm_pow[(size_t)e * PA + z_fn % PA];
+    q.b_old = F == 2 ? h.base_pow[(size_t)e * PA + z_bn % PA] : 0.f;
+    q.met = lane < WG_N_METRICS ? h.metrics[(size_t)e * WG_N_METRICS + lane] : 0.f;
     return q;
 }
 
diff --git a/windgym_amd/csrc/wg_obs.h b/windgym_amd/csrc/wg_obs.h
--- a/windgym_amd/csrc/wg_obs.h
+++ b/windgym_amd/csrc/wg_obs.h
@@ -186,18 +186,29 @@
 struct SumsEnt {
     const float* rb; int stride; bool farm; unsigned sm, cm;
 };
-template <bool TURB = false>
-__device__ __forceinline__ SumsEnt wg_sums_ent(const WgParams& p, const WgPtrs& d, const int ctx_id, const int ent) {
+template <bool TURB = false, typename P, typename D>
+__device__ __forceinline__ SumsEnt wg_sums_ent(const P& p, const D& d, const int ctx_id, const int ent) {
     SumsEnt q;
-    q.farm = TURB ? false : ent == p.N;
-    q.rb = q.farm ? d.fring + (size_t)ctx_id * p.fring_stride : d.ring + (size_t)ctx_id * p.ring_stride + ent;
-    q.stride = q.farm ? 1 : p.N;
-    q.sm = q.farm ? p.sum_mask_f : p.sum_mask_t;
-    q.cm = q.farm ? p.cur_mask_f : p.cur_mask_t;
+    if constexpr (TURB) {
+        q.farm = false;
+        q.rb = d.ring + (size_t)ctx_id * p.ring_stride + ent;
+        q.stride = p.N; q.sm = p.sum_mask_t; q.cm = p.cur_mask_t;
+    } else {
+        q.farm = ent == p.N;
+        q.rb = q.farm ? d.fring + (size_t)ctx_id * p.fring_stride : d.ring + (size_t)ctx_id * p.ring_stride + ent;
+        q.stride = q.farm ? 1 : p.N;
+        q.sm = q.farm ? p.sum_mask_f : p.sum_mask_t;
+        q.cm = q.farm ? p.cur_mask_f : p.cur_mask_t;
+    }
     return q;
 }
-template <bool GEN, bool NEWEST = true, bool TURB = false>
-__device__ inline SumsRaw wg_sums_load(const WgParams& p, const WgPtrs& d, const int e, const int ctx_id, const int ent, const int np) {
+template <bool TURB, typename P>
+__device__ __forceinline__ int wg_sums_off(const P& p, const bool farm, const int ch) {
+    if constexpr (TURB) return p.ring_off[ch];
+    else return farm ? p.fring_off[ch] : p.ring_off[ch];
+}
+template <bool GEN, bool NEWEST = true, bool TURB = false, typename P, typename D>
+__device__ inline SumsRaw wg_sums_load(const P& p, const D& d, const int e, const int ctx_id, const int ent, const int np) {
     constexpr int NSL = GEN ? WG_N_SUMS : WG_N_CH;
     SumsRaw r;
     const SumsEnt q = wg_sums_ent<TURB>(p, d, ctx_id, ent);
@@ -207,7 +218,7 @@
 #pragma unroll
     for (int ch = 0; ch < WG_N_CH; ++ch) {
         const bool need = (((q.sm | q.cm) >> ch) & 1u) || (ch == WG_CH_WS && ti);
-        const int off = q.farm ? p.fring_off[ch] : p.ring_off[ch];
+        const int off = wg_sums_off<TURB>(p, q.farm, ch);
         r.nw[ch] = (NEWEST && need) ? q.rb[off + wg_umod(np, p.ring_cap[ch], p.ring_magic[ch]) * q.stride] : 0.f;
     }
 #pragma unroll
@@ -216,7 +227,7 @@
     for (int s = 0; s < NSL; ++s) {
         if ((q.sm >> s) & 1u) {
             const int ch = s < WG_N_CH ? s : WG_CH_WS;
-            const int off = q.farm ? p.fring_off[ch] : p.ring_off[ch];
+            const int off = wg_sums_off<TURB>(p, q.farm, ch);
             const int Wc = p.sum_w[s];
             r.S[s] = ws_[(size_t)s * NS];
             if (np >= Wc) r.lv[s] = q.rb[off + wg_umod(np - Wc, p.ring_cap[ch], p.ring_magic[ch]) * q.stride];
diff --git a/windgym_amd/csrc/wg_plan.h b/windgym_amd/csrc/wg_plan.h
--- a/windgym_amd/csrc/wg_plan.h
+++ b/windgym_amd/csrc/wg_plan.h
@@ -398,6 +398,35 @@
     f.an_inv_ka = (float)(1.0 / wg_defd(c->m0_ka, 0.38));
 }
 
+inline EnvHotP wg_plan_env_hot(const FlowP& f, const FlowPtrs& d, const WgParams& gp, const WgPtrs& gd) {
+    EnvHotP h;
+    memset(&h, 0, sizeof(h));
+    EnvHotPro& a = h.pro;
+    a.env = d.env; a.slot = d.slot; a.ctx = d.ctx; a.roff = d.roff; a.xr = d.xr; a.yr = d.yr; a.yaw = d.yaw; a.u = d.u;
+    a.ti_loc = d.ti_loc; a.bnd = d.bnd; a.tab_power = d.tab_power; a.tab_ct = d.tab_ct; a.rotor_dy = d.rotor_dy; a.rotor_dz = d.rotor_dz;
+    a.N = f.N; a.F = f.F; a.inv_N = f.inv_N; a.autoreset = f.autoreset; a.K = f.K; a.n_tab = f.n_tab; a.S = f.S; a.env_inc = f.env_inc;
+    a.env_share = f.env_share;
+    EnvHotSet& s = h.set;
+    s.tab_power = d.tab_power; s.tab_ct = d.tab_ct; s.rotor_dy = d.rotor_dy; s.rotor_dz = d.rotor_dz;
+    s.env_off_tab = f.env_off_tab; s.action_method = f.action_method; s.yaw_min = f.yaw_min; s.yaw_max = f.yaw_max; s.yaw_step = f.yaw_step;
+    s.hill = f.hill; s.dt = f.dt; s.tic = f.tic; s.hub = f.hub;
+    EnvHotReq& r = h.req;
+    r.wsum = gd.wsum; r.ring = gd.ring; r.farm_pow = gd.farm_pow; r.base_pow = gd.base_pow; r.metrics = gd.metrics;
+    r.N = gp.N; r.power_avg = gp.power_avg; r.ring_stride = gp.ring_stride; r.sum_mask_t = gp.sum_mask_t; r.cur_mask_t = gp.cur_mask_t;
+    EnvHotTail& t = h.tail;
+    t.ring = d.ring; t.cur_ws = d.cur_ws; t.cur_wd = d.cur_wd; t.env = d.env;
+    t.n_tab = f.n_tab; t.tab_x0 = f.tab_x0; t.tab_inv_dx = f.tab_inv_dx; t.env_off_tab = f.env_off_tab; t.ring_stride = f.ring_stride;
+    EnvHotFarm& m = h.farm;
+    m.fring = d.fring; m.step_farm_pow = d.step_farm_pow; m.step_base_pow = d.step_base_pow; m.pend_farm = d.pend_farm; m.pend_base = d.pend_base;
+    m.fring_stride = f.fring_stride; m.power_avg = f.power_avg; m.pavg_magic = f.pavg_magic; m.inv_N = f.inv_N;
+    for (int i = 0; i < WG_N_CH; ++i) {
+        r.ring_off[i] = gp.ring_off[i]; r.sum_w[i] = gp.sum_w[i]; r.ring_cap[i] = gp.ring_cap[i]; r.ring_magic[i] = gp.ring_magic[i];
+        t.hlen[i] = f.hlen[i]; t.ring_off[i] = f.ring_off[i]; t.inv_hlen[i] = f.inv_hlen[i]; t.noise_sigma[i] = f.noise_sigma[i];
+        m.hlen[i] = f.hlen[i]; m.fring_off[i] = f.fring_off[i]; m.hmagic[i] = f.hmagic[i];
+    }
+    return h;
+}
+
 inline int wg_plan_reset_launches(const wg_config* c, const WgParams& p, int reset_chunk) {
     double xmn = 1e300, xmx = -1e300, ymn = 1e300, ymx = -1e300;
     for (int t = 0; t < p.N; ++t) {
```

Result: faster. 93.97 million (median of 6 runs) (+1.7%).
